# FishYuLi/BalancedGroupSoftmax

Measured on AMD Instinct MI355X. Metric: img/s fwd+bwd R50-FPN+BAGS 1333x800, 512 RoI (BASELINE metric: img/s/GPU fwd+bwd R50-FPN+BAGS 1333x800, 512 RoI; GroupSoftmax us/RoI), higher is better.
Workload: dtype f32 (conv/linear products on the bf16 MFMA from exact 3-way bf16 splits, fp32 accumulate: fp32-faithful)

## Files before the change

balancedgroupsoftmax_amd/capi.py:

```python
import ctypes
import os

_PKG = os.path.dirname(os.path.abspath(__file__))

c_i64p = ctypes.c_void_p
c_f32p = ctypes.c_void_p
c_ptr = ctypes.c_void_p

BGS_OK = 0
BGS_MAX_BINS = 16


class BgsLibraryError(RuntimeError):
    pass


class BgsCallError(RuntimeError):
    def __init__(self, fn, code, text):
        super().__init__('%s failed with code %d: %s' % (fn, code, text))
        self.code = code


SIGNATURES = {
    'bgs_version': (ctypes.c_int, []),
# ... 48 lines not shown
    'bgs_conv2d_dgrad_nhwc_f32': (ctypes.c_int, [c_f32p, c_f32p, c_f32p, c_f32p, c_f32p]
                                  + [ctypes.c_int] * 10 + [c_ptr]),
    'bgs_conv2d_wgrad_workspace_bytes': (ctypes.c_size_t, [ctypes.c_int] * 9),
    'bgs_conv2d_wgrad_nhwc_f32': (ctypes.c_int, [c_f32p, c_f32p, c_f32p, c_f32p]
                                  + [ctypes.c_int] * 10 + [c_ptr, c_ptr]),
    'bgs_fold_conv_bn_fwd': (ctypes.c_int, [c_f32p] * 6 + [ctypes.c_float] + [ctypes.c_int] * 5
                             + [c_f32p, c_f32p, c_ptr]),
    'bgs_fold_conv_bn_bwd': (ctypes.c_int, [c_f32p] * 7 + [ctypes.c_float] + [ctypes.c_int] * 5
                             + [c_f32p] * 4 + [c_ptr]),
    'bgs_conv2d_wgrad_bfx_workspace_bytes': (ctypes.c_size_t, [ctypes.c_int] * 9),
    'bgs_conv2d_wgrad_nhwc_f32_bfx': (ctypes.c_int, [c_f32p, c_f32p, c_f32p, c_f32p]
                                      + [ctypes.c_int] * 11 + [c_ptr, c_ptr]),
    'bgs_conv2d_wgrad_bfx_enable': (None, [ctypes.c_int]),
    'bgs_conv3x3_halo_nhwc_f32': (ctypes.c_int, [c_f32p, c_f32p, c_f32p, c_f32p] + [ctypes.c_int] * 6
                                  + [c_ptr]),
    'bgs_conv_bfx_weight_bytes': (ctypes.c_size_t, [ctypes.c_int, ctypes.c_int]),
    'bgs_conv_bfx_split_weights': (ctypes.c_int, [c_f32p, c_ptr, ctypes.c_int, ctypes.c_int, c_ptr]),
    'bgs_conv_dgrad_parity_enable': (None, [ctypes.c_int]),
    'bgs_conv_bfx_split_weights_dgrad': (ctypes.c_int, [c_f32p, c_ptr] + [ctypes.c_int] * 4 + [c_ptr]),
    'bgs_conv_bfx_workspace_bytes': (ctypes.c_size_t, [ctypes.c_longlong, ctypes.c_int, ctypes.c_int]),
    'bgs_conv2d_nhwc_f32_bfx_ws': (ctypes.c_int, [c_f32p, c_ptr, c_f32p, c_f32p, c_f32p]
                                   + [ctypes.c_int] * 12 + [c_ptr, ctypes.c_size_t, c_ptr]),
    'bgs_conv2d_dgrad_nhwc_f32_bfx_ws': (ctypes.c_int, [c_f32p, c_ptr, c_f32p, c_f32p, c_f32p]
                                         + [ctypes.c_int] * 11 + [c_ptr, ctypes.c_size_t, c_ptr]),
    'bgs_conv3x3_halo_bfx_workspace_bytes': (ctypes.c_size_t, [ctypes.c_int] * 5),
    'bgs_conv3x3_c3_fused_nhwc_f32_bfx': (ctypes.c_int, [c_f32p, c_ptr, c_f32p, c_ptr, c_f32p, c_f32p, c_f32p]
                                          + [ctypes.c_int] * 6 + [c_ptr]),
    'bgs_conv3x3_halo_nhwc_f32_bfx': (ctypes.c_int, [c_f32p, c_ptr, c_f32p, c_f32p]
                                      + [ctypes.c_int] * 7 + [c_ptr, ctypes.c_size_t, c_ptr]),
    'bgs_conv3x3_halo_nhwc_f32_bfx_ex': (ctypes.c_int, [c_f32p, c_ptr, c_f32p, c_f32p, c_f32p]
                                         + [ctypes.c_int] * 7 + [c_ptr, ctypes.c_size_t, c_ptr]),
    'bgs_conv3x3_planes_head_nhwc_f32_bfx': (ctypes.c_int, [c_f32p, c_ptr, c_f32p, c_ptr, c_f32p, c_f32p]
                                             + [ctypes.c_int] * 7 + [c_ptr]),
    'bgs_conv3x3_planes_head_eligible': (ctypes.c_int, [ctypes.c_int] * 6),
    'bgs_gs_loss_tuning': (None, [ctypes.c_int]),
    'bgs_gs_head_fold': (None, [ctypes.c_int]),
    'bgs_gs_loss_wavepriv_min_rows': (None, [ctypes.c_int]),
    'bgs_gs_merge_tuning': (None, [ctypes.c_int, ctypes.c_int]),
    'bgs_conv_bfx_wide_tuning': (None, [ctypes.c_int] * 3),
    'bgs_conv_bfx_wide_last_launch': (ctypes.c_int, []),
    'bgs_conv1x1_planes_enable': (None, [ctypes.c_int]),
    'bgs_conv1x1_planes_last_launch': (ctypes.c_int, []),
    'bgs_conv3x3_planes_enable': (None, [ctypes.c_int]),
    'bgs_conv3x3_planes_last_launch': (ctypes.c_int, []),
    'bgs_conv1x1_bres_enable': (None, [ctypes.c_int]),
    'bgs_conv1x1_bres_last_launch': (ctypes.c_int, []),
    'bgs_launch_census': (ctypes.c_int, [ctypes.c_int, ctypes.c_int]),
    'bgs_conv_bfx_tuning': (None, [ctypes.c_int] * 2),
    'bgs_conv_bfx_last_launch': (ctypes.c_int, [c_ptr, c_ptr]),
    'bgs_conv_tuning': (None, [ctypes.c_int] * 4),
    'bgs_conv_last_launch': (ctypes.c_int, [c_ptr, c_ptr, c_ptr, c_ptr]),
    'bgs_conv3x3_halo_bfx_tuning': (None, [ctypes.c_int] * 2),
    'bgs_conv3x3_halo_bfx_last_launch': (ctypes.c_int, [c_ptr, c_ptr]),
    'bgs_conv3x3_halo_bfx_last_wide': (ctypes.c_int, [c_ptr, c_ptr]),
    'bgs_conv3x3_halo_bfx_wide': (ctypes.c_int, [ctypes.c_int]),
    'bgs_grouped_conv3x3_nhwc_f32': (ctypes.c_int, [c_f32p, c_f32p, c_f32p, c_f32p] + [ctypes.c_int] * 7
                                     + [c_ptr]),
    'bgs_grouped_conv3x3_nhwc_bf16ops': (ctypes.c_int, [c_f32p, c_f32p, c_f32p, c_f32p] + [ctypes.c_int] * 7
                                         + [c_ptr]),
    'bgs_grouped_conv3x3_dgrad_nhwc_f32': (ctypes.c_int, [c_f32p, c_f32p, c_f32p] + [ctypes.c_int] * 6
                                           + [c_ptr]),
    'bgs_grouped_conv3x3_wgrad_workspace_bytes': (ctypes.c_size_t, [ctypes.c_int] * 6),
    'bgs_grouped_conv3x3_wgrad_nhwc_f32': (ctypes.c_int, [c_f32p, c_f32p, c_f32p, c_f32p]
                                           + [ctypes.c_int] * 7 + [c_ptr, c_ptr]),
    'bgs_deform_conv3x3_nhwc_f32': (ctypes.c_int, [c_f32p] * 5 + [ctypes.c_int] * 9 + [c_ptr]),
    'bgs_deform_conv3x3_dgrad_nhwc_f32': (ctypes.c_int, [c_f32p] * 6 + [ctypes.c_int] * 8 + [c_ptr]),
    'bgs_deform_conv3x3_wgrad_workspace_bytes': (ctypes.c_size_t, [ctypes.c_int] * 6),
    'bgs_deform_conv3x3_wgrad_nhwc_f32': (ctypes.c_int, [c_f32p] * 5 + [ctypes.c_int] * 9 + [c_ptr, c_ptr]),
    'bgs_sigmoid_focal_workspace_bytes': (ctypes.c_size_t, []),
    'bgs_sigmoid_focal_fwd': (ctypes.c_int, [c_f32p, ctypes.c_longlong, c_i64p, ctypes.c_int, ctypes.c_int,
                                             ctypes.c_float, ctypes.c_float, ctypes.c_int, c_f32p, c_ptr]),
    'bgs_sigmoid_focal_bwd': (ctypes.c_int, [c_f32p, ctypes.c_longlong, c_i64p, c_f32p, ctypes.c_int, ctypes.c_int,
                                             ctypes.c_float, ctypes.c_float, ctypes.c_int, c_f32p, c_ptr]),
    'bgs_sigmoid_focal_fwd_bwd': (ctypes.c_int, [c_f32p, ctypes.c_longlong, c_i64p, c_f32p, c_f32p, ctypes.c_int,
                                                 ctypes.c_int, ctypes.c_float, ctypes.c_float, ctypes.c_int, c_f32p,
                                                 ctypes.c_float, c_f32p, c_f32p, c_ptr, c_ptr]),
    'bgs_maxpool3x3s2_bwd_nhwc_f32': (ctypes.c_int, [c_f32p, c_f32p, c_f32p] + [ctypes.c_int] * 4 + [c_ptr]),
    'bgs_maxpool3x3s2_nhwc_f32': (ctypes.c_int, [c_f32p, c_f32p] + [ctypes.c_int] * 4 + [c_ptr]),
    'bgs_nchw_to_nhwc4_f32': (ctypes.c_int, [c_f32p, c_f32p] + [ctypes.c_int] * 4 + [c_ptr]),
    'bgs_conv2d_nhwc_bf16s': (ctypes.c_int, [c_ptr, c_ptr, c_f32p, c_ptr, ctypes.c_int, ctypes.c_int, c_ptr]
                              + [ctypes.c_int] * 11 + [c_ptr]),
    'bgs_grouped_conv3x3_nhwc_bf16s': (ctypes.c_int, [c_ptr, c_f32p, c_f32p, c_ptr] + [ctypes.c_int] * 7
                                       + [c_ptr]),
    'bgs_maxpool3x3s2_nhwc_f32_to_bf16': (ctypes.c_int, [c_f32p, c_ptr] + [ctypes.c_int] * 4 + [c_ptr]),
    'bgs_conv_bf16s_tuning': (None, [ctypes.c_int]),
    'bgs_roi_align_nhwc_fwd': (ctypes.c_int, [c_ptr, c_ptr, c_ptr, c_ptr, ctypes.c_int,
                                              ctypes.c_int, ctypes.c_float, c_f32p, ctypes.c_int,
                                              ctypes.c_int, ctypes.c_int, ctypes.c_int,
                                              ctypes.c_int, c_f32p, c_ptr, c_ptr]),
    'bgs_roi_align_nhwc_bwd': (ctypes.c_int, [c_ptr, c_ptr, c_ptr, c_ptr, ctypes.c_int,
                                              ctypes.c_int, ctypes.c_float, c_f32p, ctypes.c_int,
                                              ctypes.c_int, ctypes.c_int, ctypes.c_int,
                                              ctypes.c_int, c_f32p, c_ptr]),
    'bgs_roi_align_nhwc_fwd_f16': (ctypes.c_int, [c_ptr, c_ptr, c_ptr, c_ptr, ctypes.c_int,
                                                  ctypes.c_int, ctypes.c_float, c_f32p, ctypes.c_int,
                                                  ctypes.c_int, ctypes.c_int, ctypes.c_int,
                                                  ctypes.c_int, c_ptr, c_ptr, c_ptr]),
    'bgs_roi_align_nhwc_bwd_f16': (ctypes.c_int, [c_ptr, c_ptr, c_ptr, c_ptr, ctypes.c_int,
                                                  ctypes.c_int, ctypes.c_float, c_f32p, ctypes.c_int,
                                                  ctypes.c_int, ctypes.c_int, ctypes.c_int,
                                                  ctypes.c_int, c_ptr, c_ptr]),
    'bgs_roi_align_nhwc_fwd_ex': (ctypes.c_int, [c_ptr, c_ptr, c_ptr, c_ptr, ctypes.c_int,
                                                 ctypes.c_int, ctypes.c_float, c_f32p, ctypes.c_int,
                                                 ctypes.c_int, ctypes.c_int, ctypes.c_int,
                                                 ctypes.c_int, ctypes.c_int, ctypes.c_int, c_f32p,
                                                 c_ptr, c_ptr]),
    'bgs_roi_align_nhwc_bwd_ex': (ctypes.c_int, [c_ptr, c_ptr, c_ptr, c_ptr, ctypes.c_int,
                                                 ctypes.c_int, ctypes.c_float, c_f32p, ctypes.c_int,
                                                 ctypes.c_int, ctypes.c_int, ctypes.c_int,
                                                 ctypes.c_int, ctypes.c_int, c_f32p, c_ptr]),
    'bgs_resize_bilinear_nhwc_f32': (ctypes.c_int, [c_f32p, c_f32p] + [ctypes.c_int] * 7 + [c_ptr]),
    'bgs_resize_bilinear_nhwc_bwd_f32': (ctypes.c_int, [c_f32p, c_f32p] + [ctypes.c_int] * 7
                                         + [c_ptr]),
    'bgs_mask_target': (ctypes.c_int, [c_ptr, c_ptr, ctypes.c_int, ctypes.c_int, ctypes.c_int, c_f32p,
                                       ctypes.c_int, c_ptr, c_ptr, ctypes.c_int, ctypes.c_int, c_f32p,
                                       c_ptr]),
    'bgs_stem_fused_weight_bytes': (ctypes.c_size_t, []),
    'bgs_stem_fused_split_weights': (ctypes.c_int, [c_f32p, ctypes.c_int, c_ptr, c_ptr]),
    'bgs_stem_conv7x7s2_relu_maxpool_nchw_f32': (ctypes.c_int, [c_f32p, c_ptr, c_f32p, c_f32p, ctypes.c_int,
                                                                ctypes.c_int, ctypes.c_int, c_ptr]),
    'bgs_mask_paste_u8': (ctypes.c_int, [c_f32p, c_f32p, ctypes.c_int, ctypes.c_int, ctypes.c_int, ctypes.c_float,
                                         ctypes.c_float, ctypes.c_int, ctypes.c_int, c_ptr, c_ptr]),
    'bgs_mask_rle_workspace_bytes': (ctypes.c_size_t, [ctypes.c_int, ctypes.c_int]),
    'bgs_mask_rle_count': (ctypes.c_int, [c_f32p, c_f32p, ctypes.c_int, ctypes.c_int, ctypes.c_int, c_ptr, c_f32p,
                                          ctypes.c_float, ctypes.c_int, ctypes.c_int, c_ptr, ctypes.c_size_t, c_ptr,
                                          c_ptr]),
    'bgs_mask_rle_write': (ctypes.c_int, [c_f32p, c_f32p, ctypes.c_int, ctypes.c_int, ctypes.c_int, c_ptr, c_f32p,
                                          ctypes.c_float, ctypes.c_int, ctypes.c_int, c_ptr, ctypes.c_size_t, c_ptr,
                                          ctypes.c_longlong, c_ptr, c_ptr, c_ptr]),
    'bgs_rle_to_string': (ctypes.c_int, [c_ptr, c_ptr, ctypes.c_int, c_ptr, ctypes.c_longlong, c_ptr]),
    'bgs_rle_from_string': (ctypes.c_int, [c_ptr, c_ptr, ctypes.c_int, c_ptr, ctypes.c_longlong, c_ptr]),
    'bgs_lvis_box_iou': (ctypes.c_int, [c_ptr] * 5 + [ctypes.c_int] + [ctypes.c_longlong] * 3 + [c_ptr, c_ptr]),
    'bgs_lvis_rle_iou': (ctypes.c_int, [c_ptr] * 7 + [ctypes.c_int] + [ctypes.c_longlong] * 3 + [c_ptr, c_ptr]),
    'bgs_lvis_match_workspace_bytes': (ctypes.c_size_t, [ctypes.c_longlong, ctypes.c_int, ctypes.c_int]),
    'bgs_lvis_match': (ctypes.c_int, [c_ptr] * 4 + [ctypes.c_int] + [ctypes.c_longlong] * 2 + [c_ptr] * 4
                       + [c_ptr, ctypes.c_int, c_ptr, ctypes.c_int, c_ptr, ctypes.c_size_t] + [c_ptr] * 4 + [c_ptr]),
    'bgs_poly_rle_edge_points': (ctypes.c_int, [c_ptr, c_ptr, c_ptr, ctypes.c_longlong, ctypes.c_int, c_ptr, c_ptr]),
    'bgs_poly_rle_crossings': (ctypes.c_int, [c_ptr] * 4 + [ctypes.c_longlong, ctypes.c_int, ctypes.c_int, c_ptr, c_ptr,
                                              ctypes.c_longlong, c_ptr, c_ptr, c_ptr]),
    'bgs_poly_rle_events_from_transitions': (ctypes.c_int, [c_ptr] * 4 + [ctypes.c_int, ctypes.c_longlong, c_ptr,
                                                            c_ptr]),
    'bgs_poly_rle_events_from_runs': (ctypes.c_int, [c_ptr] * 3 + [ctypes.c_int, ctypes.c_longlong, c_ptr, c_ptr]),
    'bgs_poly_rle_resolve': (ctypes.c_int, [c_ptr] * 3 + [ctypes.c_int, ctypes.c_int] + [c_ptr] * 4
                             + [ctypes.c_int, ctypes.c_longlong] + [c_ptr] * 4),
    'bgs_poly_rle_write': (ctypes.c_int, [c_ptr] * 4 + [ctypes.c_int] + [c_ptr] * 4
                           + [ctypes.c_longlong, c_ptr, ctypes.c_longlong, c_ptr, c_ptr]),
    'bgs_mask_gt_logits': (ctypes.c_int, [c_f32p, c_f32p, c_f32p, c_ptr, ctypes.c_int, ctypes.c_int,
                                          ctypes.c_int, ctypes.c_int, c_f32p, c_ptr]),
    'bgs_mask_bce_partials': (ctypes.c_int, [ctypes.c_int]),
    'bgs_mask_bce': (ctypes.c_int, [c_f32p, c_f32p, c_f32p, c_ptr, c_f32p, c_ptr, c_f32p,
                                    ctypes.c_int, ctypes.c_int, ctypes.c_int, ctypes.c_int, c_f32p,
                                    c_f32p, c_f32p, c_f32p, c_ptr]),
    'bgs_topk_workspace_bytes': (ctypes.c_size_t, [ctypes.c_int, ctypes.c_int]),
    'bgs_topk_sorted_f32': (ctypes.c_int, [c_ptr, c_ptr, c_ptr, c_ptr, c_ptr, ctypes.c_int,
                                           ctypes.c_int, c_f32p, c_ptr, c_ptr, c_ptr]),
    'bgs_nms_workspace_bytes': (ctypes.c_size_t, [ctypes.c_int, ctypes.c_int]),
    'bgs_nms_batched': (ctypes.c_int, [c_f32p, c_ptr, ctypes.c_int, ctypes.c_int, ctypes.c_float,
                                       ctypes.c_int, ctypes.c_int, c_ptr, c_ptr, c_ptr, c_ptr]),
    'bgs_nms_merge_select': (ctypes.c_int, [c_f32p, c_ptr, c_ptr] + [ctypes.c_int] * 4 + [c_f32p, c_ptr, c_ptr]),
    'bgs_nms_gather': (ctypes.c_int, [c_f32p, c_ptr, c_ptr, ctypes.c_int, ctypes.c_int, c_f32p, c_f32p, c_ptr]),
    'bgs_soft_nms_batched': (ctypes.c_int, [c_f32p, c_ptr, ctypes.c_int, ctypes.c_int, ctypes.c_float, ctypes.c_int,
                                            ctypes.c_float, ctypes.c_float, c_ptr, c_f32p, c_ptr, c_ptr]),
    'bgs_det_candidates': (ctypes.c_int, [c_f32p, c_f32p, c_ptr, c_f32p] + [ctypes.c_int] * 4
                           + [ctypes.c_float, ctypes.c_int, c_f32p, c_ptr, c_ptr, c_ptr]),
    'bgs_det_select': (ctypes.c_int, [c_f32p, c_ptr, c_ptr, c_f32p, c_ptr] + [ctypes.c_int] * 4
                       + [c_f32p, c_ptr, c_ptr, c_ptr, c_ptr]),
    'bgs_gather_boxes': (ctypes.c_int, [c_f32p, c_ptr, c_f32p, ctypes.c_int, ctypes.c_int, ctypes.c_int, c_f32p,
                                        c_ptr, c_ptr]),
    'bgs_aug_map_boxes': (ctypes.c_int, [c_ptr, c_ptr] + [ctypes.c_int] * 4 + [c_ptr, c_ptr, c_ptr, ctypes.c_int,
                                                                               ctypes.c_int, c_f32p, c_f32p, c_ptr,
                                                                               c_ptr]),
    'bgs_aug_merge_bboxes': (ctypes.c_int, [c_ptr, c_ptr] + [ctypes.c_int] * 4 + [c_ptr, c_ptr, c_ptr, c_ptr, c_f32p,
                                                                                  c_f32p, c_ptr]),
    'bgs_aug_merge_masks': (ctypes.c_int, [c_ptr, c_ptr, ctypes.c_int, ctypes.c_int, ctypes.c_int, c_f32p, c_ptr]),
    'bgs_img_prep_u8': (ctypes.c_int, [c_ptr, c_ptr, ctypes.c_int, ctypes.c_int, c_f32p, ctypes.c_int, c_f32p,
                                       ctypes.c_int, ctypes.c_int, c_ptr]),
    'bgs_gt_mask_prep_u8': (ctypes.c_int, [c_ptr, c_ptr, ctypes.c_int, c_ptr, c_ptr, ctypes.c_longlong, c_ptr,
                                           ctypes.c_int, ctypes.c_int, c_ptr]),
    'bgs_gt_seg_prep_u8': (ctypes.c_int, [c_ptr, c_ptr, ctypes.c_int, c_ptr, ctypes.c_int, ctypes.c_int, c_ptr]),
    'bgs_iou_assign_workspace_bytes': (ctypes.c_size_t, [ctypes.c_int] * 3),
    'bgs_iou_assign': (ctypes.c_int, [c_f32p, ctypes.c_longlong, ctypes.c_int, c_ptr, c_f32p, c_ptr,
                                      ctypes.c_int, ctypes.c_int, ctypes.c_float, ctypes.c_float,
                                      ctypes.c_float, ctypes.c_float, c_ptr, c_f32p, c_ptr, c_ptr]),
    'bgs_rpn_loss_workspace_bytes': (ctypes.c_size_t, [ctypes.c_int] * 3),
    'bgs_rpn_loss': (ctypes.c_int, [c_ptr, c_ptr, ctypes.c_int, ctypes.c_int, c_f32p, c_ptr, c_ptr,
                                    c_ptr, c_f32p, c_ptr, ctypes.c_int, c_ptr, c_ptr,
                                    ctypes.c_float, ctypes.c_float, ctypes.c_float, ctypes.c_float,
                                    c_f32p, c_f32p, c_f32p, c_ptr, c_ptr]),
    'bgs_rpn_loss_grad': (ctypes.c_int, [c_ptr, c_ptr, c_ptr, ctypes.c_int, ctypes.c_int, c_f32p,
                                         c_ptr, c_ptr, c_ptr, c_f32p, c_ptr, ctypes.c_int, c_ptr,
                                         c_ptr, ctypes.c_float, ctypes.c_float, ctypes.c_float,
                                         ctypes.c_float, c_f32p, c_f32p, c_f32p, c_ptr]),
    'bgs_sample_pos_neg_workspace_bytes': (ctypes.c_size_t, [ctypes.c_int]),
    'bgs_sample_pos_neg': (ctypes.c_int, [c_ptr, ctypes.c_int, ctypes.c_int, ctypes.c_int, ctypes.c_float,
                                          ctypes.c_float, ctypes.c_uint64, c_ptr, c_ptr, c_ptr, c_ptr,
                                          c_ptr]),
    'bgs_sample_rois': (ctypes.c_int, [c_ptr, c_ptr, ctypes.c_int, ctypes.c_int, ctypes.c_float,
                                       ctypes.c_uint64, c_ptr, c_ptr, c_ptr, c_ptr, c_ptr]),
    'bgs_sample_rois_ex': (ctypes.c_int, [c_ptr, c_ptr, c_ptr, ctypes.c_int, ctypes.c_int, ctypes.c_float,
                                          ctypes.c_uint64, c_ptr, c_ptr, c_ptr, c_ptr, c_ptr, c_ptr, c_ptr]),
    'bgs_random_keys': (ctypes.c_int, [ctypes.c_uint64, c_ptr, ctypes.c_int, c_ptr, c_ptr]),
    'bgs_decode_proposals': (ctypes.c_int, [c_ptr, c_ptr, c_ptr, ctypes.c_int, ctypes.c_int, c_f32p,
                                            c_ptr, c_f32p, ctypes.c_int, c_ptr, c_ptr, c_ptr,
                                            ctypes.c_float, ctypes.c_int, c_f32p, c_ptr]),
    'bgs_refine_boxes': (ctypes.c_int, [c_f32p, c_ptr, c_f32p, ctypes.c_int, ctypes.c_int, c_ptr,
                                        ctypes.c_int, c_f32p, c_f32p, ctypes.c_float, c_f32p, c_ptr]),
    'bgs_rcnn_targets': (ctypes.c_int, [c_ptr, c_ptr, c_ptr, c_ptr, c_ptr, c_ptr, c_f32p, c_ptr,
                                        ctypes.c_int, ctypes.c_int, c_ptr, c_ptr, ctypes.c_float,
                                        c_f32p, c_ptr, c_f32p, c_f32p, c_f32p, c_ptr]),
}

_LIB = None


def lib_filename():
    variant = os.environ.get('BGS_LIB_VARIANT', '')
    return 'libbgs_%s.so' % variant if variant else 'libbgs.so'


def lib_path():
    return os.environ.get('BGS_LIB_PATH', os.path.join(_PKG, lib_filename()))


def load():
    global _LIB
    if _LIB is not None:
        return _LIB
    path = lib_path()
    if not os.path.exists(path):
        raise BgsLibraryError(
            '%s not found. Build the HIP kernels first: '
            '`python -m balancedgroupsoftmax_amd.csrc.build` (or __graft_entry__.build()). '
            'There is deliberately no CPU fallback.' % path)
    try:
        lib = ctypes.CDLL(path)
    except OSError as e:
        raise BgsLibraryError('cannot load %s: %s' % (path, e))
    for name, (res, args) in SIGNATURES.items():
        try:
            fn = getattr(lib, name)
        except AttributeError:
            raise BgsLibraryError('%s does not export %s (stale build?)' % (path, name))
        fn.restype = res
        fn.argtypes = args
    _LIB = lib
    return lib


def check(fn_name, code):
    if code != BGS_OK:
        raise BgsCallError(fn_name, code, load().bgs_error_string(code).decode())


def host_i64(a):
    import numpy as np
    a = np.ascontiguousarray(a, dtype=np.int64)
    return a, a.ctypes.data_as(ctypes.c_void_p)


def ptr(t):
    return None if t is None else t.data_ptr()


_RAW_STREAM = []


def raw_stream(device=None):
    import torch
    if not _RAW_STREAM:
        _RAW_STREAM.append(getattr(torch._C, '_cuda_getCurrentRawStream', None))
    idx = device if isinstance(device, int) else getattr(device, 'index', None)
    if idx is None:
        if isinstance(device, str):
            idx = torch.device(device).index
        if idx is None:
            idx = torch.cuda.current_device()
    fn = _RAW_STREAM[0]
    if fn is None:
        return torch.cuda.current_stream(idx).cuda_stream
    return fn(idx)


def current_stream(device=None):
    return raw_stream(device)
```

balancedgroupsoftmax_amd/csrc/det_targets.hip:

```cpp
#include <math.h>
#include <string.h>

#include "bgs_common.h"

namespace {

constexpr int kMaxImgs = 16;
constexpr int kMaxLevels = 8;
constexpr int kGtChunk = 256;

struct ImgTable {
  int gt_off[kMaxImgs + 1];
  int img_h[kMaxImgs], img_w[kMaxImgs];
};

__device__ __forceinline__ float iou1(float ax1, float ay1, float ax2, float ay2, float aarea,
                                      float bx1, float by1, float bx2, float by2) {
#pragma clang fp contract(off)
  const float w = fmaxf(fminf(ax2, bx2) - fmaxf(ax1, bx1) + 1.f, 0.f);
  const float h = fmaxf(fminf(ay2, by2) - fmaxf(ay1, by1) + 1.f, 0.f);
  const float ov = w * h;
  const float barea = (bx2 - bx1 + 1.f) * (by2 - by1 + 1.f);
  return ov / (barea + aarea - ov);
}
// ... 310 lines not shown
  const size_t row = ((size_t)n * Lv.hw[lvl] + loc) * ch;
  const float* o = Lv.out[lvl] + row;
  float* d_o = G.dout[lvl] + row;
  const float inv = 1.f / num_total[0];
  const float x = o[a];
  const float t = ps ? 1.f : 0.f;
  const float w = ps ? pos_weight : 1.f;
  const float sig = 1.f / (1.f + expf(-x));
  d_o[a] = g_cls[lvl] * w_cls * w * (sig - t) * inv;
  if (ps) {
    const int g = T.gt_off[n] + assigned[(size_t)n * A + i] - 1;
    const float* an = anchors + (size_t)i * 4;
    const float* gb = gt + (size_t)g * 4;
    float d[4];
    encode_delta(an[0], an[1], an[2], an[3], gb[0], gb[1], gb[2], gb[3], cod, d);
    const float sc = g_bbox[lvl] * w_bbox * inv;
#pragma unroll
    for (int c = 0; c < 4; ++c) {
      const float df = o[na + a * 4 + c] - d[c];
      const float ad = fabsf(df);
      const float gr = ad < beta ? df / beta : (df > 0.f ? 1.f : (df < 0.f ? -1.f : 0.f));
      d_o[na + a * 4 + c] = sc * gr;
    }
  }
}

struct CountTable {
  int count[kMaxLevels];
};

__global__ __launch_bounds__(256) void decode_proposals_kernel(
    LevelTable Lv, ImgTable T, CountTable Ct, const float* __restrict__ anchors,
    const long long* __restrict__ top_idx, const float* __restrict__ top_logit, Coding cod,
    float max_ratio, int nmax, float* __restrict__ boxes_out) {
  const int n = blockIdx.z, l = blockIdx.y;
  const int j = blockIdx.x * 256 + threadIdx.x;
  if (j >= nmax) return;
  float* o = boxes_out + (((size_t)n * Lv.num_levels + l) * nmax + j) * 5;
  if (j >= Ct.count[l]) {
    o[0] = o[1] = o[2] = o[3] = o[4] = 0.f;
    return;
  }
  const size_t tj = ((size_t)n * Lv.num_levels + l) * nmax + j;
  long long p = top_idx[tj];
  const int na = Lv.num_anchors, ch = 5 * na;
  const long long cnt = (long long)Lv.hw[l] * na;
  p = p < 0 ? 0 : (p >= cnt ? cnt - 1 : p);
  const int loc = (int)(p / na), a = (int)(p - (long long)loc * na);
  const float* src = Lv.out[l] + ((size_t)n * Lv.hw[l] + loc) * ch + na + a * 4;
  const float* an = anchors + ((size_t)Lv.start[l] + p) * 4;
  const float dx = src[0] * cod.stdv[0] + cod.mean[0];
  const float dy = src[1] * cod.stdv[1] + cod.mean[1];
  float dw = src[2] * cod.stdv[2] + cod.mean[2];
  float dh = src[3] * cod.stdv[3] + cod.mean[3];
  dw = fminf(fmaxf(dw, -max_ratio), max_ratio);
  dh = fminf(fmaxf(dh, -max_ratio), max_ratio);
  const float px = (an[0] + an[2]) * 0.5f, py = (an[1] + an[3]) * 0.5f;
  const float pw = an[2] - an[0] + 1.f, ph = an[3] - an[1] + 1.f;
  const float gw = pw * expf(dw), gh = ph * expf(dh);
  const float gx = px + pw * dx, gy = py + ph * dy;
  const float wmax = (float)(T.img_w[n] - 1), hmax = (float)(T.img_h[n] - 1);
  o[0] = fminf(fmaxf(gx - gw * 0.5f + 0.5f, 0.f), wmax);
  o[1] = fminf(fmaxf(gy - gh * 0.5f + 0.5f, 0.f), hmax);
  o[2] = fminf(fmaxf(gx + gw * 0.5f - 0.5f, 0.f), wmax);
  o[3] = fminf(fmaxf(gy + gh * 0.5f - 0.5f, 0.f), hmax);
  o[4] = 1.f / (1.f + expf(-top_logit[tj]));
}

__global__ __launch_bounds__(256) void refine_boxes_kernel(const float* __restrict__ rois,
                                                           const long long* __restrict__ labels,
                                                           const float* __restrict__ bbox_pred,
                                                           int K, int pred_cols, Coding cod,
                                                           ImgTable T, int n_img, float max_ratio,
                                                           float* __restrict__ out) {
#pragma clang fp contract(off)
  const int k = blockIdx.x * 256 + threadIdx.x;
  if (k >= K) return;
  const float* r = rois + (size_t)k * 5;
  int img = (int)r[0];
  img = img < 0 ? 0 : (img >= n_img ? n_img - 1 : img);
  long long c = 0;
  if (pred_cols > 4 && labels) {
    c = labels[k];
    const long long nc = pred_cols / 4;
    c = c < 0 ? 0 : (c >= nc ? nc - 1 : c);
  }
  const float* d = bbox_pred + (size_t)k * pred_cols + c * 4;
  const float dx = d[0] * cod.stdv[0] + cod.mean[0];
  const float dy = d[1] * cod.stdv[1] + cod.mean[1];
  float dw = d[2] * cod.stdv[2] + cod.mean[2];
  float dh = d[3] * cod.stdv[3] + cod.mean[3];
  dw = fminf(fmaxf(dw, -max_ratio), max_ratio);
  dh = fminf(fmaxf(dh, -max_ratio), max_ratio);
  const float pw = r[3] - r[1] + 1.0f, ph = r[4] - r[2] + 1.0f;
  const float px = (r[1] + r[3]) * 0.5f, py = (r[2] + r[4]) * 0.5f;
  const float gw = pw * expf(dw), gh = ph * expf(dh);
  const float gx = px + pw * dx, gy = py + ph * dy;
  const float wmax = (float)(T.img_w[img] - 1), hmax = (float)(T.img_h[img] - 1);
  float* o = out + (size_t)k * 4;
  o[0] = fminf(fmaxf(gx - gw * 0.5f + 0.5f, 0.f), wmax);
  o[1] = fminf(fmaxf(gy - gh * 0.5f + 0.5f, 0.f), hmax);
  o[2] = fminf(fmaxf(gx + gw * 0.5f - 0.5f, 0.f), wmax);
  o[3] = fminf(fmaxf(gy + gh * 0.5f - 0.5f, 0.f), hmax);
}

struct PtrTable {
  const float* boxes[kMaxImgs];
  const int* assigned[kMaxImgs];
  const long long* inds[kMaxImgs];
  const uint8_t* valid[kMaxImgs];
  const long long* gt_labels[kMaxImgs];
  int box_stride[kMaxImgs];
};

__global__ __launch_bounds__(256) void rcnn_targets_kernel(PtrTable P, ImgTable T,
                                                           const float* __restrict__ gt, Coding cod,
                                                           int num, float pos_weight,
                                                           float* __restrict__ rois,
                                                           long long* __restrict__ labels,
                                                           float* __restrict__ label_weights,
                                                           float* __restrict__ bbox_targets,
                                                           float* __restrict__ bbox_weights) {
  const int n = blockIdx.y;
  const int j = blockIdx.x * 256 + threadIdx.x;
  if (j >= num) return;
  const size_t r = (size_t)n * num + j;
  const long long ci = P.inds[n][j];
  const float* b = P.boxes[n] + (size_t)ci * P.box_stride[n];
  const int a = P.assigned[n][ci];
  const bool ok = P.valid[n] ? P.valid[n][j] != 0 : true;
  const bool pos = ok && a > 0;
  rois[r * 5 + 0] = (float)n;
  rois[r * 5 + 1] = b[0];
  rois[r * 5 + 2] = b[1];
  rois[r * 5 + 3] = b[2];
  rois[r * 5 + 4] = b[3];
  float d[4] = {0.f, 0.f, 0.f, 0.f};
  long long lab = 0;
  if (pos) {
    const int g = T.gt_off[n] + (int)a - 1;
    const float* gb = gt + (size_t)g * 4;
    encode_delta(b[0], b[1], b[2], b[3], gb[0], gb[1], gb[2], gb[3], cod, d);
    lab = P.gt_labels[n][a - 1];
  }
  labels[r] = lab;
  label_weights[r] = pos ? pos_weight : (ok ? 1.f : 0.f);
#pragma unroll
  for (int c = 0; c < 4; ++c) {
    bbox_targets[r * 4 + c] = d[c];
    bbox_weights[r * 4 + c] = pos ? 1.f : 0.f;
  }
}

int fill_img_table(ImgTable* T, const int* host_gt_offsets, const int* host_img_hw, int N) {
  if (N <= 0 || N > kMaxImgs || !host_gt_offsets) return BGS_ERR_INVALID_ARG;
  for (int i = 0; i <= kMaxImgs; ++i) T->gt_off[i] = 0;
  for (int i = 0; i <= N; ++i) T->gt_off[i] = host_gt_offsets[i];
  for (int i = 0; i < kMaxImgs; ++i) {
    T->img_h[i] = host_img_hw ? host_img_hw[2 * (i < N ? i : 0)] : 1;
    T->img_w[i] = host_img_hw ? host_img_hw[2 * (i < N ? i : 0) + 1] : 1;
  }
  for (int i = 0; i < N; ++i)
    if (T->gt_off[i + 1] < T->gt_off[i]) return BGS_ERR_INVALID_ARG;
  return BGS_OK;
}

int fill_level_table(LevelTable* Lv, const float* const* host_outs, const int* host_hw, int L,
                     int num_anchors) {
  if (L <= 0 || L > kMaxLevels || !host_outs || !host_hw || num_anchors <= 0)
    return BGS_ERR_INVALID_ARG;
  int start = 0;
  for (int l = 0; l < kMaxLevels; ++l) {
    Lv->out[l] = l < L ? host_outs[l] : nullptr;
    Lv->hw[l] = l < L ? host_hw[l] : 0;
    Lv->start[l] = start;
    if (l < L) {
      if (!host_outs[l] || host_hw[l] <= 0) return BGS_ERR_INVALID_ARG;
      start += host_hw[l] * num_anchors;
    }
  }
  Lv->start[kMaxLevels] = start;
  for (int l = L; l <= kMaxLevels; ++l) Lv->start[l] = start;
  Lv->num_levels = L;
  Lv->num_anchors = num_anchors;
  return BGS_OK;
}

}

extern "C" size_t bgs_iou_assign_workspace_bytes(int N, int A, int G_total) {
  if (N <= 0 || A <= 0 || G_total < 0) return 0;
  const size_t g = (size_t)(G_total > 0 ? G_total : 1);
  return (size_t)N * A * 4 + (size_t)N * g * 4 + (size_t)N * ((A + 255) / 256) * g * 4;
}

extern "C" int bgs_iou_assign(const float* boxes, long long box_img_stride, int box_stride,
                              const uint8_t* valid,
                              const float* gt, const int* host_gt_offsets, int N, int A,
                              float pos_iou_thr, float neg_iou_lo, float neg_iou_hi,
                              float min_pos_iou, int* assigned, float* max_overlaps_out,
                              void* workspace, bgs_stream_t stream) {
  if (N <= 0 || A <= 0 || !boxes || !gt || !assigned || !workspace || box_stride < 4)
    return BGS_ERR_INVALID_ARG;
  ImgTable T;
  const int rc = fill_img_table(&T, host_gt_offsets, nullptr, N);
  if (rc != BGS_OK) return rc;
  const int Gt = T.gt_off[N];
  if (Gt <= 0) return BGS_ERR_INVALID_ARG;
  hipStream_t st = (hipStream_t)stream;
  float* box_max = max_overlaps_out;
  int* gt_max = (int*)((char*)workspace + (size_t)N * A * 4);
  int* blk_max = gt_max + (size_t)N * Gt;
  const size_t ng = (size_t)N * Gt;
  hipLaunchKernelGGL(fill_i32_kernel, dim3((unsigned)((ng + 255) / 256)), dim3(256), 0, st, gt_max,
                     (int)0xBF800000 , ng);
  dim3 grid((unsigned)((A + 255) / 256), (unsigned)N);
  const float send = min_pos_iou > 0.f ? min_pos_iou : 0.f;
  int send_bits;
  memcpy(&send_bits, &send, sizeof(int));
  hipLaunchKernelGGL(iou_gtmax_kernel, grid, dim3(256), 0, st, boxes, box_img_stride, box_stride,
                     valid, gt, T, A, Gt, pos_iou_thr, neg_iou_lo, neg_iou_hi, send_bits, box_max, blk_max,
                     gt_max, assigned);
  hipLaunchKernelGGL(iou_assign_kernel, grid, dim3(256), 0, st, boxes, box_img_stride, box_stride,
                     valid, gt, T, A, Gt, blk_max, gt_max, min_pos_iou, assigned);
  BGS_RETURN_LAUNCH_STATUS();
}

extern "C" size_t bgs_rpn_loss_workspace_bytes(int N, int A_total, int L) {
  if (N <= 0 || A_total <= 0 || L <= 0) return 0;
  return (size_t)N * ((A_total + 255) / 256) * L * 4 * sizeof(float);
}

extern "C" int bgs_rpn_loss(const float* const* host_level_outs, const int* host_level_hw, int L,
                            int num_anchors, const float* anchors, const int* assigned,
                            const uint8_t* pos_mask, const uint8_t* neg_mask, const float* gt,
                            const int* host_gt_offsets, int N, const float* host_means,
                            const float* host_stds, float beta, float pos_weight,
                            float loss_weight_cls, float loss_weight_bbox, float* loss_cls_out,
                            float* loss_bbox_out, float* num_total_out, void* workspace,
                            bgs_stream_t stream) {
  if (!anchors || !assigned || !pos_mask || !neg_mask || !gt || !loss_cls_out || !loss_bbox_out ||
      !workspace || !host_means || !host_stds || !(beta > 0.f))
    return BGS_ERR_INVALID_ARG;
  LevelTable Lv;
  int rc = fill_level_table(&Lv, host_level_outs, host_level_hw, L, num_anchors);
  if (rc != BGS_OK) return rc;
  ImgTable T;
  rc = fill_img_table(&T, host_gt_offsets, nullptr, N);
  if (rc != BGS_OK) return rc;
  Coding cod;
  for (int c = 0; c < 4; ++c) {
    cod.mean[c] = host_means[c];
    cod.stdv[c] = host_stds[c];
  }
  const int A = Lv.start[kMaxLevels];
  const int blocks = (A + 255) / 256;
  hipStream_t st = (hipStream_t)stream;
  hipLaunchKernelGGL(rpn_loss_kernel, dim3(blocks, N), dim3(256), 0, st, Lv, T, anchors, assigned,
                     pos_mask, neg_mask, gt, cod, beta, pos_weight <= 0.f ? 1.f : pos_weight, A,
                     (float*)workspace);
  hipLaunchKernelGGL(rpn_loss_finalize_kernel, dim3(1), dim3(1024), 0, st, (const float*)workspace,
                     Lv, N, blocks, L, loss_weight_cls, loss_weight_bbox, loss_cls_out, loss_bbox_out,
                     num_total_out);
  BGS_RETURN_LAUNCH_STATUS();
}

__global__ __launch_bounds__(256) void random_keys_kernel(uint64_t seed,
                                                          const long long* __restrict__ draw, int n,
                                                          long long* __restrict__ out) {
  const int i = blockIdx.x * 256 + threadIdx.x;
  if (i >= n) return;
  const uint64_t d = draw ? (uint64_t)draw[0] : 0ull;
  uint64_t x = seed + 0x9E3779B97F4A7C15ull * ((uint64_t)i + 1ull) + 0xD1B54A32D192ED03ull * (d + 1ull);
  x ^= x >> 30; x *= 0xBF58476D1CE4E5B9ull;
  x ^= x >> 27; x *= 0x94D049BB133111EBull;
  x ^= x >> 31;
  out[i] = (long long)(x >> 2);
}

extern "C" int bgs_random_keys(uint64_t seed, const long long* draw_counter, int n, long long* out,
                               bgs_stream_t stream) {
  if (n < 0) return BGS_ERR_INVALID_ARG;
  if (n == 0) return BGS_OK;
  if (!out) return BGS_ERR_INVALID_ARG;
  hipLaunchKernelGGL(random_keys_kernel, dim3((n + 255) / 256), dim3(256), 0, (hipStream_t)stream,
                     seed, draw_counter, n, out);
  BGS_RETURN_LAUNCH_STATUS();
}

extern "C" int bgs_rpn_loss_grad(const float* const* host_level_outs,
                                 float* const* host_level_douts, const int* host_level_hw, int L,
                                 int num_anchors, const float* anchors, const int* assigned,
                                 const uint8_t* pos_mask, const uint8_t* neg_mask, const float* gt,
                                 const int* host_gt_offsets, int N, const float* host_means,
                                 const float* host_stds, float beta, float pos_weight,
                                 float loss_weight_cls, float loss_weight_bbox,
                                 const float* num_total, const float* grad_loss_cls,
                                 const float* grad_loss_bbox, bgs_stream_t stream) {
  if (!anchors || !assigned || !pos_mask || !neg_mask || !gt || !num_total || !grad_loss_cls ||
      !grad_loss_bbox || !host_level_douts || !host_means || !host_stds || !(beta > 0.f))
    return BGS_ERR_INVALID_ARG;
  LevelTable Lv;
  int rc = fill_level_table(&Lv, host_level_outs, host_level_hw, L, num_anchors);
  if (rc != BGS_OK) return rc;
  GradTable G;
  for (int l = 0; l < kMaxLevels; ++l) G.dout[l] = nullptr;
  for (int l = 0; l < L; ++l) {
    if (!host_level_douts[l]) return BGS_ERR_INVALID_ARG;
    G.dout[l] = host_level_douts[l];
  }
  ImgTable T;
  rc = fill_img_table(&T, host_gt_offsets, nullptr, N);
  if (rc != BGS_OK) return rc;
  Coding cod;
  for (int c = 0; c < 4; ++c) {
    cod.mean[c] = host_means[c];
    cod.stdv[c] = host_stds[c];
  }
  const int A = Lv.start[kMaxLevels];
  const int blocks = (A + 255) / 256;
  hipLaunchKernelGGL(rpn_loss_grad_kernel, dim3(blocks, N), dim3(256), 0, (hipStream_t)stream, Lv,
                     G, T, anchors, assigned, pos_mask, neg_mask, gt, cod, beta,
                     pos_weight <= 0.f ? 1.f : pos_weight, A, num_total, loss_weight_cls,
                     loss_weight_bbox, grad_loss_cls, grad_loss_bbox);
  BGS_RETURN_LAUNCH_STATUS();
}

extern "C" int bgs_decode_proposals(const float* const* host_level_outs, const int* host_level_hw,
                                    const int* host_level_counts, int L, int num_anchors,
                                    const float* anchors, const long long* top_idx,
                                    const float* top_logit, int N, const int* host_img_hw,
                                    const float* host_means, const float* host_stds,
                                    float wh_ratio_clip, int nmax, float* boxes_out,
                                    bgs_stream_t stream) {
  if (!anchors || !top_idx || !top_logit || !boxes_out || !host_img_hw || !host_means ||
      !host_stds || !host_level_counts || nmax <= 0 || !(wh_ratio_clip > 0.f))
    return BGS_ERR_INVALID_ARG;
  LevelTable Lv;
  int rc = fill_level_table(&Lv, host_level_outs, host_level_hw, L, num_anchors);
  if (rc != BGS_OK) return rc;
  ImgTable T;
  int zero_off[kMaxImgs + 1] = {0};
  rc = fill_img_table(&T, zero_off, host_img_hw, N);
  if (rc != BGS_OK) return rc;
  Coding cod;
  CountTable Ct;
  for (int c = 0; c < 4; ++c) {
    cod.mean[c] = host_means[c];
    cod.stdv[c] = host_stds[c];
  }
  for (int l = 0; l < kMaxLevels; ++l) Ct.count[l] = l < L ? host_level_counts[l] : 0;
  hipLaunchKernelGGL(decode_proposals_kernel, dim3((nmax + 255) / 256, L, N), dim3(256), 0,
                     (hipStream_t)stream, Lv, T, Ct, anchors, top_idx, top_logit, cod,
                     fabsf(logf(wh_ratio_clip)), nmax, boxes_out);
  BGS_RETURN_LAUNCH_STATUS();
}

extern "C" int bgs_refine_boxes(const float* rois, const long long* labels, const float* bbox_pred,
                                int K, int pred_cols, const int* host_img_hw, int N,
                                const float* host_means, const float* host_stds, float wh_ratio_clip,
                                float* out, bgs_stream_t stream) {
  if (K < 0 || N <= 0 || N > kMaxImgs || pred_cols < 4 || pred_cols % 4 != 0) return BGS_ERR_INVALID_ARG;
  if (K == 0) return BGS_OK;
  if (!rois || !bbox_pred || !out || !host_img_hw || !host_means || !host_stds || wh_ratio_clip <= 0.f)
    return BGS_ERR_INVALID_ARG;
  if (pred_cols > 4 && !labels) return BGS_ERR_INVALID_ARG;
  ImgTable T;
  for (int i = 0; i < kMaxImgs; ++i) {
    const int s = i < N ? i : 0;
    T.gt_off[i] = 0;
    T.img_h[i] = host_img_hw[2 * s];
    T.img_w[i] = host_img_hw[2 * s + 1];
  }
  T.gt_off[kMaxImgs] = 0;
  Coding cod;
  for (int i = 0; i < 4; ++i) {
    cod.mean[i] = host_means[i];
    cod.stdv[i] = host_stds[i];
  }
  hipLaunchKernelGGL(refine_boxes_kernel, dim3((K + 255) / 256), dim3(256), 0, (hipStream_t)stream, rois,
                     labels, bbox_pred, K, pred_cols, cod, T, N, fabsf(logf(wh_ratio_clip)), out);
  BGS_RETURN_LAUNCH_STATUS();
}

extern "C" int bgs_rcnn_targets(const float* const* host_boxes, const int* host_box_strides,
                                const int* const* host_assigned,
                                const long long* const* host_inds,
                                const uint8_t* const* host_valid,
                                const long long* const* host_gt_labels, const float* gt,
                                const int* host_gt_offsets, int N, int num, const float* host_means,
                                const float* host_stds, float pos_weight, float* rois,
                                long long* labels, float* label_weights, float* bbox_targets,
                                float* bbox_weights, bgs_stream_t stream) {
  if (!host_boxes || !host_box_strides || !host_assigned || !host_inds || !host_gt_labels || !gt ||
      !rois || !labels || !label_weights || !bbox_targets || !bbox_weights || num <= 0 ||
      !host_means || !host_stds)
    return BGS_ERR_INVALID_ARG;
  ImgTable T;
  const int rc = fill_img_table(&T, host_gt_offsets, nullptr, N);
  if (rc != BGS_OK) return rc;
  PtrTable P;
  for (int i = 0; i < kMaxImgs; ++i) {
    const int s = i < N ? i : 0;
    P.boxes[i] = host_boxes[s];
    P.assigned[i] = host_assigned[s];
    P.inds[i] = host_inds[s];
    P.valid[i] = host_valid ? host_valid[s] : nullptr;
    P.gt_labels[i] = host_gt_labels[s];
    P.box_stride[i] = host_box_strides[s];
    if (i < N && (!P.boxes[i] || !P.assigned[i] || !P.inds[i] || !P.gt_labels[i] ||
                  P.box_stride[i] < 4))
      return BGS_ERR_INVALID_ARG;
  }
  Coding cod;
  for (int c = 0; c < 4; ++c) {
    cod.mean[c] = host_means[c];
    cod.stdv[c] = host_stds[c];
  }
  hipLaunchKernelGGL(rcnn_targets_kernel, dim3((num + 255) / 256, N), dim3(256), 0,
                     (hipStream_t)stream, P, T, gt, cod, num, pos_weight <= 0.f ? 1.f : pos_weight,
                     rois, labels, label_weights, bbox_targets, bbox_weights);
  BGS_RETURN_LAUNCH_STATUS();
}
```

balancedgroupsoftmax_amd/csrc/topk.hip:

```cpp
#include "bgs_common.h"

namespace {

constexpr int kMaxProblems = 64;
constexpr int kMaxK = 4096;
constexpr int kBins = 2048;
constexpr int kChunk = 4096;
constexpr int kState = 8;

struct TopkProblems {
  const float* row[kMaxProblems];
  int len[kMaxProblems];
  int k[kMaxProblems];
  int inner[kMaxProblems];
  int pitch[kMaxProblems];
};

__device__ __forceinline__ float topk_elem(const TopkProblems& pr, int p, const float* row, int i) {
  const int inner = pr.inner[p];
  if (inner == 0) return row[i];
  const int q = i / inner;
  return row[(size_t)q * pr.pitch[p] + (i - q * inner)];
}

struct TopkWs {
  int* hist;
  unsigned* state;
  unsigned long long* list;
};

__device__ __forceinline__ unsigned key_of(float f) {
  const unsigned b = __float_as_uint(f);
  return (b & 0x80000000u) ? ~b : (b | 0x80000000u);
}
__device__ __forceinline__ float value_of(unsigned key) {
  return __uint_as_float((key & 0x80000000u) ? (key & 0x7fffffffu) : ~key);
}

__device__ __forceinline__ int shift_of(int pass) { return pass == 0 ? 21 : (pass == 1 ? 10 : 0); }
__device__ __forceinline__ int bins_of(int pass) { return pass == 2 ? 1024 : 2048; }

__device__ __forceinline__ void topk_pick(const int* __restrict__ g, int nb, int k_rem, int* s_wave, int* s_res,
                                          int& digit, int& k_in) {
  const int tid = threadIdx.x, lane = tid & 63, wave = tid >> 6;
  const int per = nb / 256;
  int cnt[8];
  int mine = 0;
#pragma unroll
  for (int j = 0; j < 8; ++j) {
    cnt[j] = j < per ? g[nb - 1 - (tid * per + j)] : 0;
    mine += cnt[j];
  }
  int incl = mine;
#pragma unroll
  for (int off = 1; off < 64; off <<= 1) {
    const int t = __shfl_up(incl, off, 64);
    if (lane >= off) incl += t;
  }
  if (lane == 63) s_wave[wave] = incl;
  __syncthreads();
  int base = 0;
  for (int w = 0; w < wave; ++w) base += s_wave[w];
  incl += base;
  const int excl = incl - mine;
  if (excl < k_rem && k_rem <= incl) {
    int c = excl, d = 0;
#pragma unroll
    for (int j = 0; j < 8; ++j) {
      if (j < per) {
        if (k_rem <= c + cnt[j]) {
          d = nb - 1 - (tid * per + j);
          break;
        }
        c += cnt[j];
      }
    }
    s_res[0] = d;
    s_res[1] = k_rem - c;
  }
  __syncthreads();
  digit = s_res[0];
  k_in = s_res[1];
  __syncthreads();
}

__global__ __launch_bounds__(256) void topk_hist_kernel(TopkProblems pr, TopkWs ws, int pass) {
  __shared__ int h[kBins];
  __shared__ int s_wave[4], s_res[2];
  const int p = blockIdx.y, tid = threadIdx.x;
  const int len = pr.len[p];
  const int lo = blockIdx.x * kChunk;
  if (lo >= len) return;
  const int hi = min(len, lo + kChunk);
  const int k = min(pr.k[p], len);
  if (k <= 0) return;
  const int nb = bins_of(pass), shift = shift_of(pass);
  for (int b = tid; b < nb; b += 256) h[b] = 0;
  unsigned* st = ws.state + p * kState;
  unsigned prefix = 0, pmask = 0;
  if (pass > 0) {
    int k_rem = k;
    if (pass == 2) {
      prefix = st[0];
      pmask = st[1];
      k_rem = (int)st[2];
    }
    int digit, k_in;
    topk_pick(ws.hist + ((size_t)p * 3 + (pass - 1)) * kBins, bins_of(pass - 1), k_rem, s_wave, s_res, digit, k_in);
    prefix |= (unsigned)digit << shift_of(pass - 1);
    pmask |= (unsigned)(bins_of(pass - 1) - 1) << shift_of(pass - 1);
    if (blockIdx.x == 0 && tid == 0) {
      unsigned* o = st + (pass == 1 ? 0 : 5);
      o[0] = prefix;
      o[1] = pmask;
      o[2] = (unsigned)k_in;
    }
  }
  __syncthreads();
  const float* row = pr.row[p];
  for (int i = lo + tid; i < hi; i += 256) {
    const unsigned key = key_of(topk_elem(pr, p, row, i));
    if ((key & pmask) == prefix) atomicAdd(&h[(key >> shift) & (nb - 1)], 1);
  }
  __syncthreads();
  int* g = ws.hist + ((size_t)p * 3 + pass) * kBins;
  for (int b = tid; b < nb; b += 256)
    if (h[b]) atomicAdd(&g[b], h[b]);
}

__global__ __launch_bounds__(256) void topk_collect_kernel(TopkProblems pr, TopkWs ws, int kmax) {
  const int p = blockIdx.y, tid = threadIdx.x;
  const int len = pr.len[p];
  const int lo = blockIdx.x * kChunk;
  if (lo >= len) return;
  const int hi = min(len, lo + kChunk);
  const int k = min(pr.k[p], len);
  unsigned* st = ws.state + p * kState;
  unsigned long long* list = ws.list + (size_t)p * kmax;
  const float* row = pr.row[p];
  if (k <= 0) return;
  __shared__ int s_wave[4], s_res[2];
  int digit, need_eq;
  topk_pick(ws.hist + ((size_t)p * 3 + 2) * kBins, bins_of(2), (int)st[7], s_wave, s_res, digit, need_eq);
  const unsigned T = st[5] | ((unsigned)digit << shift_of(2));
  const int lane = tid & 63;
  const unsigned long long below = (1ull << lane) - 1ull;
  constexpr int kLg = 512, kLe = 256;
  __shared__ unsigned long long s_g[kLg], s_e[kLe];
  __shared__ int s_n[2], s_base[2];
  if (tid < 2) s_n[tid] = 0;
  __syncthreads();
  for (int i0 = lo; i0 < hi; i0 += 256) {
    const int i = i0 + tid;
    const bool in = i < hi;
    const unsigned key = in ? key_of(topk_elem(pr, p, row, i)) : 0u;
    const unsigned long long comp = ((unsigned long long)key << 32) | (0xffffffffu - (unsigned)i);
    const bool gt = in && key > T, eq = in && key == T;
    const unsigned long long mg = __ballot(gt), me = __ballot(eq);
    if (mg) {
      const int leader = __ffsll((long long)mg) - 1;
      int base = 0;
      if (lane == leader) base = atomicAdd(&s_n[0], __popcll(mg));
      base = __shfl(base, leader, 64);
      const int slot = base + __popcll(mg & below);
      if (gt) {
        if (slot < kLg) s_g[slot] = comp;
        else list[atomicAdd(&st[3], 1u)] = comp;
      }
    }
    if (me) {
      const int leader = __ffsll((long long)me) - 1;
      int base = 0;
      if (lane == leader) base = atomicAdd(&s_n[1], __popcll(me));
      base = __shfl(base, leader, 64);
      const int slot = base + __popcll(me & below);
      if (eq) {
        if (slot < kLe) s_e[slot] = comp;
        else {
          const int g = (int)atomicAdd(&st[4], 1u);
          if (g < need_eq) list[k - 1 - g] = comp;
        }
      }
    }
  }
  __syncthreads();
  const int ng = min(s_n[0], kLg), ne = min(s_n[1], kLe);
  if (tid == 0) {
    s_base[0] = ng ? (int)atomicAdd(&st[3], (unsigned)ng) : 0;
    s_base[1] = ne ? (int)atomicAdd(&st[4], (unsigned)ne) : 0;
  }
  __syncthreads();
  for (int i = tid; i < ng; i += 256) list[s_base[0] + i] = s_g[i];
  for (int i = tid; i < ne; i += 256) {
    const int g = s_base[1] + i;
    if (g < need_eq) list[k - 1 - g] = s_e[i];
  }
}

__global__ __launch_bounds__(1024) void topk_sort_kernel(TopkProblems pr, TopkWs ws, int kmax,
                                                         float* __restrict__ out_val,
                                                         long long* __restrict__ out_idx) {
  __shared__ unsigned long long buf[kMaxK];
  const int p = blockIdx.x, tid = threadIdx.x;
  const int k = min(pr.k[p], pr.len[p]);
  int m = 1;
  while (m < k) m <<= 1;
  const unsigned long long* list = ws.list + (size_t)p * kmax;
  for (int i = tid; i < m; i += 1024) buf[i] = i < k ? list[i] : 0ull;
  __syncthreads();
  for (int size = 2; size <= m; size <<= 1) {
    for (int stride = size >> 1; stride > 0; stride >>= 1) {
      for (int j = tid; j < (m >> 1); j += 1024) {
        const int lo = (j / stride) * (stride << 1) + (j % stride);
        const int hi = lo + stride;
        const bool desc = ((lo & size) == 0);
        const unsigned long long a = buf[lo], b = buf[hi];
        if ((a < b) == desc) {
          buf[lo] = b;
          buf[hi] = a;
        }
      }
      bgs::bitonic_stage_sync(size, stride);
    }
  }
  __syncthreads();
  float* ov = out_val + (size_t)p * kmax;
  long long* oi = out_idx + (size_t)p * kmax;
  for (int i = tid; i < kmax; i += 1024) {
    if (i < k) {
      const unsigned long long c = buf[i];
      ov[i] = value_of((unsigned)(c >> 32));
      oi[i] = (long long)(0xffffffffu - (unsigned)(c & 0xffffffffu));
    } else {
      ov[i] = 0.f;
      oi[i] = 0;
    }
  }
}

}

extern "C" size_t bgs_topk_workspace_bytes(int P, int kmax) {
  if (P <= 0 || kmax <= 0) return 0;
  return (size_t)P * (3 * kBins * sizeof(int) + kState * sizeof(unsigned) +
                      (size_t)kmax * sizeof(unsigned long long));
}

extern "C" int bgs_topk_sorted_f32(const float* const* host_rows, const int* host_len,
                                   const int* host_k, const int* host_inner,
                                   const int* host_pitch, int P, int kmax, float* out_val,
                                   long long* out_idx, void* workspace, bgs_stream_t stream) {
  if (P < 0 || kmax <= 0) return BGS_ERR_INVALID_ARG;
  if (P == 0) return BGS_OK;
  if (!host_rows || !host_len || !host_k || !out_val || !out_idx || !workspace)
    return BGS_ERR_INVALID_ARG;
  if (P > kMaxProblems || kmax > kMaxK) return BGS_ERR_UNSUPPORTED;
  TopkProblems pr;
  int maxlen = 0;
  for (int p = 0; p < kMaxProblems; ++p) {
    pr.row[p] = nullptr;
    pr.len[p] = pr.k[p] = pr.inner[p] = pr.pitch[p] = 0;
  }
  if ((host_inner == nullptr) != (host_pitch == nullptr)) return BGS_ERR_INVALID_ARG;
  for (int p = 0; p < P; ++p) {
    if (host_len[p] < 0 || host_k[p] < 0 || host_k[p] > kmax) return BGS_ERR_INVALID_ARG;
    if (host_len[p] > 0 && !host_rows[p]) return BGS_ERR_INVALID_ARG;
    pr.row[p] = host_rows[p];
    pr.len[p] = host_len[p];
    pr.k[p] = host_k[p];
    if (host_inner) {
      if (host_inner[p] < 0 || (host_inner[p] > 0 && host_pitch[p] < host_inner[p]))
        return BGS_ERR_INVALID_ARG;
      pr.inner[p] = host_inner[p];
      pr.pitch[p] = host_pitch[p];
    }
    if (host_len[p] > maxlen) maxlen = host_len[p];
  }
  TopkWs ws;
  ws.hist = reinterpret_cast<int*>(workspace);
  ws.state = reinterpret_cast<unsigned*>(ws.hist + (size_t)P * 3 * kBins);
  ws.list = reinterpret_cast<unsigned long long*>(ws.state + (size_t)P * kState);
  hipStream_t st = (hipStream_t)stream;
  if (hipMemsetAsync(workspace, 0, (size_t)P * (3 * kBins * sizeof(int) + kState * sizeof(unsigned)),
                     st) != hipSuccess)
    return BGS_ERR_LAUNCH;
  const int G = maxlen > 0 ? (maxlen + kChunk - 1) / kChunk : 1;
  for (int pass = 0; pass < 3; ++pass)
    hipLaunchKernelGGL(topk_hist_kernel, dim3(G, P), dim3(256), 0, st, pr, ws, pass);
  hipLaunchKernelGGL(topk_collect_kernel, dim3(G, P), dim3(256), 0, st, pr, ws, kmax);
  hipLaunchKernelGGL(topk_sort_kernel, dim3(P), dim3(1024), 0, st, pr, ws, kmax, out_val, out_idx);
  BGS_RETURN_LAUNCH_STATUS();
}
```

balancedgroupsoftmax_amd/detectors.py:

```python
import torch
import torch.nn as nn

from . import box_ops, builder, merge_augs
from . import functional as BF
from . import post_processing as PP
from .registry import DETECTORS


_GT_ROWS = {}


def _gt_index_row(G, device):
    key = (int(G), str(device))
    t = _GT_ROWS.get(key)
    if t is None:
        if len(_GT_ROWS) > 4096:
            _GT_ROWS.clear()
        t = _GT_ROWS[key] = torch.arange(1, int(G) + 1, device=device, dtype=torch.int32)
    return t


@DETECTORS.register_module
class TwoStageDetector(nn.Module):

    def __init__(self, backbone, neck=None, shared_head=None, rpn_head=None,
                 bbox_roi_extractor=None, bbox_head=None, mask_roi_extractor=None, mask_head=None,
                 train_cfg=None, test_cfg=None, pretrained=None):
        super().__init__()
        if shared_head is not None:
            raise NotImplementedError('shared_head (C4 heads) is not on the BAGS path')
        self.backbone = builder.build_backbone(backbone)
        self.neck = builder.build_neck(neck) if neck is not None else None
        self.rpn_head = builder.build_head(rpn_head) if rpn_head is not None else None
        self.bbox_roi_extractor = builder.build_roi_extractor(bbox_roi_extractor) \
            if bbox_head is not None else None
        self.bbox_head = builder.build_head(bbox_head) if bbox_head is not None else None
        self.mask_head = None
        if mask_head is not None:
            if mask_roi_extractor is not None:
                self.mask_roi_extractor = builder.build_roi_extractor(mask_roi_extractor)
                self.share_roi_extractor = False
            else:
                self.share_roi_extractor = True
                self.mask_roi_extractor = self.bbox_roi_extractor
            self.mask_head = builder.build_head(mask_head)
        self.train_cfg, self.test_cfg = train_cfg, test_cfg
        self.fp16_enabled = False
        self.init_weights(pretrained=pretrained)

    with_neck = property(lambda self: self.neck is not None)
    with_rpn = property(lambda self: self.rpn_head is not None)
    with_bbox = property(lambda self: self.bbox_head is not None)
    with_mask = property(lambda self: self.mask_head is not None)
    with_shared_head = property(lambda self: False)

    def init_weights(self, pretrained=None):
        self.backbone.init_weights(pretrained=pretrained)
        if self.with_neck:
            self.neck.init_weights()
        if self.with_rpn:
            self.rpn_head.init_weights()
        if self.with_bbox:
            self.bbox_roi_extractor.init_weights()
            self.bbox_head.init_weights()
        if self.with_mask:
            self.mask_head.init_weights()
            if not self.share_roi_extractor:
                self.mask_roi_extractor.init_weights()

    def extract_feat(self, img):
        x = self.backbone(img)
        return self.neck(x) if self.with_neck else x

    def _sample_rois_fused(self, proposal_list, gt_bboxes, gt_labels, samplers=None, rc=None,
                           head=None):
        rc = self.train_cfg.rcnn if rc is None else rc
        ac, sc = rc.assigner, rc.sampler
        N = len(proposal_list)
        if hasattr(proposal_list, 'batched'):
            props, pv = proposal_list.batched
            props = props.contiguous()
            pvalid = (pv.view(torch.uint8) if pv.dtype == torch.bool else pv.to(torch.uint8)).contiguous()
        else:
            props = torch.stack([p for p, _ in proposal_list]).contiguous()
            pvalid = torch.stack([v for _, v in proposal_list]).to(torch.uint8).contiguous()
        gt_cat = torch.cat([g[:, :4] for g in gt_bboxes]).float().contiguous()
        offs = [0]
        for g in gt_bboxes:
            offs.append(offs[-1] + int(g.size(0)))
        assigned = BF.iou_assign(props, gt_cat, offs, ac.pos_iou_thr, ac.neg_iou_thr,
                                 ac.get('min_pos_iou', 0.0), valid=pvalid, shared_boxes=False)
        add_gt = sc.get('add_gt_as_proposals', True)
        rcnn_hook = samplers.get('rcnn') if samplers else None
        boxes_l, assigned_l, inds_l, valid_l = [], [], [], []
        for i in range(N):
            b, a = props[i, :, :4], assigned[i]
            if add_gt:
                G = gt_bboxes[i].size(0)
                b = torch.cat([gt_bboxes[i][:, :4].float(), b], 0)
                a = torch.cat([_gt_index_row(G, a.device), a])
            boxes_l.append(b.contiguous())
            assigned_l.append(a.contiguous())
            if rcnn_hook is not None:
                inds, _, valid = rcnn_hook(a, sc.num, sc.pos_fraction)
                inds_l.append(inds.contiguous())
                valid_l.append(valid)
        if rcnn_hook is None:
            if any(a.numel() > 4096 for a in assigned_l):
                raise NotImplementedError('bgs_sample_rois sorts <= 4096 candidates per image in LDS '
                                          '(rpn_proposal.max_num + GT boxes)')
            need_extra = self.with_mask or isinstance(self.bbox_head, nn.ModuleList)
            res = BF.sample_rois(assigned_l, sc.num, sc.pos_fraction,
                                 gt_counts=[int(g.size(0)) if add_gt else 0 for g in gt_bboxes]
                                 if need_extra else None)
            inds_all, valid_all = res[0], res[2].view(torch.bool)
            inds_l = [inds_all[i] for i in range(N)]
            valid_l = [valid_all[i] for i in range(N)]
            if need_extra:
                self._sampled_gt_inds = res[3]
                self._sampled_valid = valid_all
                self._sampled_is_gt = res[4].view(torch.bool)
        if rcnn_hook is not None and (self.with_mask or isinstance(self.bbox_head, nn.ModuleList)):
            self._sampled_gt_inds = torch.stack(
                [assigned_l[i].gather(0, inds_l[i]).to(torch.int32) - 1 for i in range(N)])
            self._sampled_valid = torch.stack(valid_l)
            self._sampled_is_gt = torch.stack(
                [(inds_l[i] < gt_bboxes[i].size(0)) if add_gt else torch.zeros_like(valid_l[i])
                 for i in range(N)])
        head = self.bbox_head if head is None else head
        rois, labels, lw, bt, bw = BF.rcnn_targets(
            boxes_l, assigned_l, inds_l, valid_l, [g.contiguous() for g in gt_labels], gt_cat, offs,
            sc.num, head.target_means, head.target_stds, rc.pos_weight)
        return rois, (labels, lw, bt, bw)

    def _rpn_forward_train(self, x, img_meta, gt_bboxes, proposals, samplers, losses, fork_loss=False):
        if not self.with_rpn:
            return [(p, torch.ones(p.size(0), dtype=torch.bool, device=p.device)) for p in proposals]
        cls_scores, bbox_preds = self.rpn_head(x)
        self._rpn_loss_fork = None
        if fork_loss and cls_scores[0].is_cuda and BF.rpn_loss_fork_enabled() and not samplers and \
                not (torch.is_grad_enabled() and cls_scores[0].requires_grad):
            with BF.forked(cls_scores[0].device, lane=1) as fk:
                losses.update(self.rpn_head.loss(cls_scores, bbox_preds, gt_bboxes, img_meta,
                                                 self.train_cfg.rpn, samplers=samplers))
            fk.hold(cls_scores, bbox_preds, self.rpn_head._fused, gt_bboxes)
            self._rpn_loss_fork = fk
        else:
            losses.update(self.rpn_head.loss(cls_scores, bbox_preds, gt_bboxes, img_meta,
                                             self.train_cfg.rpn, samplers=samplers))
        proposal_cfg = self.train_cfg.get('rpn_proposal', None)
        if proposal_cfg is None:
            proposal_cfg = self.test_cfg.rpn
        proposal_list = self.rpn_head.get_bboxes(cls_scores, bbox_preds, img_meta, proposal_cfg)
        if samplers is not None and 'proposals' in samplers:
            self._own_proposals = proposal_list
            proposal_list = samplers['proposals'](proposal_list)
        self.rpn_head._fused = None
        return proposal_list

    def _join_rpn_loss(self):
        fk = getattr(self, '_rpn_loss_fork', None)
        if fk is not None:
            fk.join()
            self._rpn_loss_fork = None

    def trunk_is_frozen(self):
        mods = [self.backbone] + ([self.neck] if self.with_neck else [])
        return not any(p.requires_grad for m in mods for p in m.parameters())

    def forward_train(self, img, img_meta, gt_bboxes, gt_labels, gt_bboxes_ignore=None,
                      gt_masks=None, proposals=None, samplers=None, feats=None):
        x = self.extract_feat(img) if feats is None else feats
        losses = dict()
        proposal_list = self._rpn_forward_train(x, img_meta, gt_bboxes, proposals, samplers, losses,
                                                fork_loss=True)
        if self.with_bbox:
            if not self.train_cfg.rcnn.assigner.get('gt_max_assign_all', True):
                raise NotImplementedError('gt_max_assign_all=False')
            rois, targets = self._sample_rois_fused(proposal_list, gt_bboxes, gt_labels, samplers)
            mask_fk = None
            if self.with_mask and rois.is_cuda and BF.rpn_loss_fork_enabled() and not (
                    torch.is_grad_enabled() and any(p.requires_grad for p in self.mask_head.parameters())):
                with BF.forked(rois.device, lane=2) as mask_fk:
                    mask_losses = self._mask_forward_train(x, rois, targets[0], gt_masks, img.size(0))
                mask_fk.hold(x, rois, targets, gt_masks)
            bbox_feats = self.bbox_roi_extractor(x[:self.bbox_roi_extractor.num_inputs], rois)
            cls_score, bbox_pred = self.bbox_head(bbox_feats, nhwc=True, reg_labels=targets[0])
            losses.update(self.bbox_head.loss(cls_score, bbox_pred, *targets))
            if mask_fk is not None:
                mask_fk.join()
                losses.update(mask_losses)
            elif self.with_mask:
                losses.update(self._mask_forward_train(x, rois, targets[0], gt_masks, img.size(0)))
        elif self.with_mask:
            losses.update(self._mask_forward_train(x, rois, targets[0], gt_masks, img.size(0)))
        self._join_rpn_loss()
        return losses

    def _mask_forward_train(self, x, rois, labels, gt_masks, num_imgs):
        if gt_masks is None:
            raise ValueError('the mask branch needs gt_masks (per image a uint8 [G, H, W] tensor)')
        if not rois.is_cuda:
            raise NotImplementedError('the mask branch runs on the GPU path only')
        sc = self.train_cfg.rcnn.sampler
        max_pos = int(sc.num * sc.pos_fraction)
        num = sc.num
        sel = (torch.arange(num_imgs, device=rois.device).view(-1, 1) * num +
               torch.arange(max_pos, device=rois.device).view(1, -1)).reshape(-1)
        pos_rois = rois[sel].contiguous()
        pos_labels = labels[sel].contiguous()
        valid = pos_labels > 0
        gt_inds = self._sampled_gt_inds[:, :max_pos].reshape(-1).contiguous()
        masks = [torch.as_tensor(m).to(device=rois.device, dtype=torch.uint8).contiguous()
                 for m in gt_masks]
        if self.share_roi_extractor:
            raise NotImplementedError('share_roi_extractor=True (7x7 features for the mask head) '
                                      'is not used by the BAGS configs')
        mask_feats = self.mask_roi_extractor(x[:self.mask_roi_extractor.num_inputs], pos_rois)
        feats = self.mask_head.features(mask_feats, nhwc=True)
        mask_targets = self.mask_head.get_target_fixed(pos_rois, gt_inds, valid, masks,
                                                       self.train_cfg.rcnn)
        return self.mask_head.loss_from_features(feats, mask_targets, pos_labels, valid)

    _last_bbox_head = property(lambda self: self.bbox_head)
    _segm_head = property(lambda self: self.mask_head)

    def _check_test_cfg(self):
        """What the detector's test_cfg asks for and is not built (raised before any device work)."""

    def _test_context(self, x):
        return None

    def _box_scores(self, x, ctx, rois, img_metas, batched=False):
        feats = self.bbox_roi_extractor(x[:self.bbox_roi_extractor.num_inputs], rois)
        return (rois,) + tuple(self.bbox_head(feats, nhwc=True))

    def _stage_mask_probs(self, x, ctx, rois, labels):
        feats = self.mask_roi_extractor(x[:self.mask_roi_extractor.num_inputs], rois)
        return [self.mask_head.get_mask_probs(self.mask_head.features(feats, nhwc=True), labels)]

    def _mask_probs(self, x, ctx, rois, labels):
        if rois.shape[0] == 0:
            return rois.new_zeros((0, 28, 28))
        probs = self._stage_mask_probs(x, ctx, rois, labels)
        return probs[0] if len(probs) == 1 else sum(probs) / float(len(probs))

    @staticmethod
    def _image_proposals(proposal_list, as_rois=True):
        props, valid = proposal_list[0] if isinstance(proposal_list[0], tuple) else (proposal_list[0], None)
        if as_rois:
            props = torch.cat([props.new_zeros((props.size(0), 1)), props[:, :4]], dim=1)
        return props, valid

    @staticmethod
    def _check_segm(segm):
        if segm not in (None, 'rle'):
            raise ValueError("segm: None (mask probabilities) or 'rle' (the reference's segm_results), got %r" % (segm,))
        return segm is not None

    def simple_test_rpn(self, x, img_meta, rpn_test_cfg):
        cls_scores, bbox_preds = self.rpn_head(x)
        return self.rpn_head.get_bboxes(cls_scores, bbox_preds, img_meta, rpn_test_cfg)

    def simple_test_bboxes(self, x, img_meta, proposals, rcnn_test_cfg, rescale=False, ctx=None):
        rois, valid = self._image_proposals(proposals)
        rois, cls_score, bbox_pred = self._box_scores(x, ctx, rois, img_meta)
        bboxes, scores = self._last_bbox_head.get_det_bboxes(
            rois, cls_score, bbox_pred, img_meta[0]['img_shape'], img_meta[0]['scale_factor'],
            rescale=rescale, cfg=None)
        if valid is not None:
            scores = torch.where(valid[:, None], scores, scores.new_full((), -1.0))
        det_bboxes, det_labels = PP.multiclass_nms(bboxes, scores, rcnn_test_cfg.score_thr,
                                                   rcnn_test_cfg.nms, rcnn_test_cfg.max_per_img)
        return det_bboxes, det_labels, scores

    def simple_test_mask(self, x, img_meta, det_bboxes, det_labels, rescale=False, paste=False, encode=None,
                         ctx=None):
        if paste and det_bboxes.shape[0] == 0:
            return [[] for _ in range(self._segm_head.num_classes - 1)]
        boxes = det_bboxes[:, :4] * img_meta[0]['scale_factor'] if rescale else det_bboxes[:, :4]
        rois = torch.cat([boxes.new_zeros((boxes.size(0), 1)), boxes], dim=1)
        probs = self._mask_probs(x, ctx, rois, det_labels)
# ... 477 lines not shown
```

balancedgroupsoftmax_amd/functional.py:

```python
import ctypes
import itertools
import os

import torch

from . import capi

_WS = {}


def _workspace(nbytes, device):
    key = (device.index, capi.raw_stream(device))
    buf = _WS.get(key)
    if buf is None or buf.numel() < nbytes:
        buf = torch.empty(max(int(nbytes), 1 << 20), dtype=torch.uint8, device=device)
        _WS[key] = buf
    return buf


def reset_workspaces():
    _WS.clear()


_SIDE = {}
# ... 1514 lines not shown
    _require_cuda(rois, *feats)
    lib = capi.load()
    L = len(feats)
    N, _, _, C = feats[0].shape
    for f in feats:
        assert f.dtype == torch.float32 and f.is_contiguous() and f.shape[0] == N and f.shape[3] == C
    rois = _f32c(rois)
    K = rois.shape[0]
    ph, pw = (out_size, out_size) if isinstance(out_size, int) else tuple(out_size)
    accumulate = out is not None
    if accumulate:
        assert tuple(out.shape) == (K, ph, pw, C) and out.is_contiguous() and \
            out.dtype == torch.float32, (out.shape, (K, ph, pw, C))
    else:
        out = torch.empty((K, ph, pw, C), dtype=torch.float32, device=rois.device)
    lv = torch.empty((K,), dtype=torch.int32, device=rois.device) if return_levels else None
    ptrs = (ctypes.c_void_p * L)(*[f.data_ptr() for f in feats])
    hs = (ctypes.c_int * L)(*[int(f.shape[1]) for f in feats])
    ws = (ctypes.c_int * L)(*[int(f.shape[2]) for f in feats])
    sc = (ctypes.c_float * L)(*[1.0 / s for s in featmap_strides])
    rc = lib.bgs_roi_align_nhwc_fwd_ex(ptrs, hs, ws, sc, L, N, float(finest_scale), capi.ptr(rois),
                                       K, C, ph, pw, sample_num, int(pool), int(accumulate),
                                       capi.ptr(out), capi.ptr(lv),
                                       capi.current_stream(rois.device))
    capi.check('bgs_roi_align_nhwc_fwd_ex', rc)
    return (out, lv) if return_levels else out


def roi_align_nhwc_bwd(dout, rois, dfeats, featmap_strides, sample_num=2, finest_scale=56, pool=1):
    import ctypes
    _require_cuda(dout, rois, *dfeats)
    lib = capi.load()
    L = len(dfeats)
    N, _, _, C = dfeats[0].shape
    for f in dfeats:
        assert f.dtype == torch.float32 and f.is_contiguous() and f.shape[0] == N and f.shape[3] == C
    rois = _f32c(rois)
    dout = _f32c(dout)
    K, ph, pw, C2 = dout.shape
    assert C2 == C and rois.shape[0] == K
    ptrs = (ctypes.c_void_p * L)(*[f.data_ptr() for f in dfeats])
    hs = (ctypes.c_int * L)(*[int(f.shape[1]) for f in dfeats])
    ws = (ctypes.c_int * L)(*[int(f.shape[2]) for f in dfeats])
    sc = (ctypes.c_float * L)(*[1.0 / s for s in featmap_strides])
    rc = lib.bgs_roi_align_nhwc_bwd_ex(ptrs, hs, ws, sc, L, N, float(finest_scale), capi.ptr(rois),
                                       K, C, ph, pw, sample_num, int(pool), capi.ptr(dout),
                                       capi.current_stream(rois.device))
    capi.check('bgs_roi_align_nhwc_bwd_ex', rc)
    return dfeats


class _RoIAlignFn(torch.autograd.Function):

    @staticmethod
    def forward(ctx, rois, strides, out_size, sample_num, finest_scale, pool, base, *feats):
        ctx.save_for_backward(rois)
        ctx.cfg = (tuple(strides), sample_num, finest_scale, pool, [tuple(f.shape) for f in feats],
                   base is not None)
        if base is not None:
            ctx.mark_dirty(base)
        return roi_align_nhwc([f.detach() for f in feats], rois, strides, out_size, sample_num,
                              finest_scale, pool=pool, out=base)

    @staticmethod
    @torch.autograd.function.once_differentiable
    def backward(ctx, dout):
        rois, = ctx.saved_tensors
        strides, sample_num, finest_scale, pool, shapes, has_base = ctx.cfg
        dout = dout.contiguous()
        dfeats = [None] * len(shapes)
        if any(ctx.needs_input_grad[7:]):
            dfeats = [torch.zeros(s, dtype=torch.float32, device=dout.device) for s in shapes]
            roi_align_nhwc_bwd(dout, rois, dfeats, strides, sample_num, finest_scale, pool=pool)
        dbase = dout if has_base and ctx.needs_input_grad[6] else None
        return (None, None, None, None, None, None, dbase) + tuple(dfeats)


def roi_align_nhwc_autograd(feats, rois, featmap_strides, out_size=7, sample_num=2,
                            finest_scale=56, pool=1, add_to=None):
    ts = list(feats) + ([add_to] if add_to is not None else [])
    if torch.is_grad_enabled() and any(t.requires_grad for t in ts):
        return _RoIAlignFn.apply(rois, tuple(featmap_strides), out_size, sample_num, finest_scale,
                                 pool, add_to, *feats)
    return roi_align_nhwc(feats, rois, featmap_strides, out_size, sample_num, finest_scale,
                          pool=pool, out=add_to)


def resize_bilinear_nhwc(x, size):
    _require_cuda(x)
    lib = capi.load()
    assert x.dtype == torch.float32 and x.is_contiguous() and x.dim() == 4
    N, H, W, C = x.shape
    Ho, Wo = int(size[0]), int(size[1])
    y = torch.empty((N, Ho, Wo, C), dtype=torch.float32, device=x.device)
    rc = lib.bgs_resize_bilinear_nhwc_f32(capi.ptr(x), capi.ptr(y), N, H, W, C, Ho, Wo, 1,
                                          capi.current_stream(x.device))
    capi.check('bgs_resize_bilinear_nhwc_f32', rc)
    return y


class _ResizeBilinearFn(torch.autograd.Function):

    @staticmethod
    def forward(ctx, x, size):
        ctx.in_shape = tuple(x.shape)
        return resize_bilinear_nhwc(x.detach(), size)

    @staticmethod
    @torch.autograd.function.once_differentiable
    def backward(ctx, dy):
        lib = capi.load()
        N, H, W, C = ctx.in_shape
        dy = dy.contiguous()
        dx = torch.zeros(ctx.in_shape, dtype=torch.float32, device=dy.device)
        rc = lib.bgs_resize_bilinear_nhwc_bwd_f32(capi.ptr(dy), capi.ptr(dx), N, H, W, C,
                                                  dy.shape[1], dy.shape[2], 1,
                                                  capi.current_stream(dy.device))
        capi.check('bgs_resize_bilinear_nhwc_bwd_f32', rc)
        return dx, None


def resize_bilinear_nhwc_autograd(x, size):
    if torch.is_grad_enabled() and x.requires_grad:
        return _ResizeBilinearFn.apply(x, tuple(size))
    return resize_bilinear_nhwc(x, size)


def topk_sorted(rows, ks, kmax, inner=None):
    import ctypes
    _require_cuda(*rows)
    lib = capi.load()
    N = rows[0].shape[0]
    L = len(rows)
    dev = rows[0].device
    ptrs, lens, kk, inn, pit = [], [], [], [], []
    for i in range(N):
        for r, k in zip(rows, ks):
            assert r.shape[0] == N and r.dtype == torch.float32 and r.is_contiguous()
            per = r[0].numel()
            ptrs.append(r.data_ptr() + i * per * 4)
            if inner is None:
                lens.append(per)
                inn.append(0)
                pit.append(0)
            else:
                C = int(r.shape[-1])
                lens.append(per // C * int(inner))
                inn.append(int(inner))
                pit.append(C)
            kk.append(int(k))
    P = N * L
    vals = torch.empty((N, L, kmax), dtype=torch.float32, device=dev)
    idx = torch.empty((N, L, kmax), dtype=torch.int64, device=dev)
    ws = _workspace(lib.bgs_topk_workspace_bytes(P, int(kmax)), dev)
    rc = lib.bgs_topk_sorted_f32((ctypes.c_void_p * P)(*ptrs), _c_int_array(lens), _c_int_array(kk),
                                 _c_int_array(inn) if inner is not None else None,
                                 _c_int_array(pit) if inner is not None else None,
                                 P, int(kmax), capi.ptr(vals), capi.ptr(idx), capi.ptr(ws),
                                 capi.current_stream(dev))
    capi.check('bgs_topk_sorted_f32', rc)
    return vals, idx


def nms_batched(boxes, counts, iou_thr, iou_mode=0, max_keep=0):
    _require_cuda(boxes, counts)
    lib = capi.load()
    boxes = _f32c(boxes)
    assert boxes.dim() == 3 and boxes.shape[2] == 5 and counts.dtype == torch.int32
    P, nmax, _ = boxes.shape
    dev = boxes.device
    keep = torch.empty((P, nmax), dtype=torch.int32, device=dev)
    keep_count = torch.empty((P,), dtype=torch.int32, device=dev)
    ws = _workspace(lib.bgs_nms_workspace_bytes(P, nmax), dev)
    rc = lib.bgs_nms_batched(capi.ptr(boxes), capi.ptr(counts), P, nmax, float(iou_thr),
                             int(iou_mode), int(max_keep), capi.ptr(keep), capi.ptr(keep_count),
                             capi.ptr(ws), capi.current_stream(dev))
    capi.check('bgs_nms_batched', rc)
    return keep, keep_count


SOFT_NMS_METHODS = {'hard': 0, 'linear': 1, 'gaussian': 2}


def soft_nms_batched(dets, counts, iou_thr, method='linear', sigma=0.5, min_score=1e-3):
    _require_cuda(dets, counts)
    code = SOFT_NMS_METHODS.get(method, method)
    if code not in (0, 1, 2):
        raise ValueError('Invalid method for SoftNMS: {}'.format(method))
    lib = capi.load()
    dets = _f32c(dets)
    assert dets.dim() == 3 and dets.shape[2] == 5 and counts.dtype == torch.int32
    P, nmax, _ = dets.shape
    dev = dets.device
    order = torch.empty((P, nmax), dtype=torch.int32, device=dev)
    scores = torch.empty((P, nmax), dtype=torch.float32, device=dev)
    keep_count = torch.empty((P,), dtype=torch.int32, device=dev)
    rc = lib.bgs_soft_nms_batched(capi.ptr(dets), capi.ptr(counts.contiguous()), P, nmax, float(iou_thr), int(code),
                                  float(sigma), float(min_score), capi.ptr(order), capi.ptr(scores),
                                  capi.ptr(keep_count), capi.current_stream(dev))
    capi.check('bgs_soft_nms_batched', rc)
    return order, scores, keep_count


DET_CANDIDATE_MODES = {'sorted': 0, 'original': 1}
DET_SELECT_WORKSPACE_PER_IMAGE = 65536


def det_candidates(scores, boxes, score_thr, mode='sorted', valid=None, score_factors=None, out=None):
    _require_cuda(scores, boxes, valid, score_factors)
    code = DET_CANDIDATE_MODES.get(mode, mode)
    if code not in (0, 1):
        raise ValueError('det_candidates: mode must be "sorted" or "original" (got %r)' % (mode,))
    lib = capi.load()
    assert scores.dim() == 3 and boxes.dim() == 3 and scores.dtype == torch.float32 and boxes.dtype == torch.float32
    B, n, C = scores.shape
    assert boxes.shape[:2] == (B, n) and boxes.shape[2] in (4, 4 * C) and C >= 2 and n >= 1 and B >= 1
    scores, boxes = scores.detach().contiguous(), boxes.detach().contiguous()
    if valid is not None:
        assert valid.shape == (B, n) and valid.dtype in (torch.bool, torch.uint8)
        valid = valid.contiguous().view(torch.uint8)
    if score_factors is not None:
        assert score_factors.shape == (B, n)
        score_factors = _f32c(score_factors)
    dev = scores.device
    P = B * (C - 1)
    if out is None:
        out = (torch.empty((P, n, 5), dtype=torch.float32, device=dev),
               torch.empty((P, n), dtype=torch.int32, device=dev),
               torch.empty((P,), dtype=torch.int32, device=dev))
    dets, idx, counts = out
    assert dets.shape == (P, n, 5) and dets.dtype == torch.float32 and dets.is_contiguous()
    assert idx.shape == (P, n) and idx.dtype == torch.int32 and idx.is_contiguous()
    assert counts.shape == (P,) and counts.dtype == torch.int32
    rc = lib.bgs_det_candidates(capi.ptr(scores), capi.ptr(boxes), capi.ptr(valid) if valid is not None else None,
                                capi.ptr(score_factors) if score_factors is not None else None, B, n, C,
                                int(boxes.shape[2]), float(score_thr), int(code), capi.ptr(dets), capi.ptr(idx),
                                capi.ptr(counts), capi.current_stream(dev))
    capi.check('bgs_det_candidates', rc)
    return dets, idx, counts


def det_select(dets, idx, keep, keep_count, num_imgs, max_num, sel_scores=None, out=None):
    _require_cuda(dets, idx, keep, keep_count, sel_scores)
    lib = capi.load()
    assert dets.dim() == 3 and dets.shape[2] == 5 and dets.dtype == torch.float32 and dets.is_contiguous()
    P, n, _ = dets.shape
    B = int(num_imgs)
    assert B >= 1 and P % B == 0 and int(max_num) > 0
    for t in (idx, keep):
        assert t.shape == (P, n) and t.dtype == torch.int32 and t.is_contiguous()
    assert keep_count.shape == (P,) and keep_count.dtype == torch.int32
    if sel_scores is not None:
        assert sel_scores.shape == (P, n) and sel_scores.dtype == torch.float32 and sel_scores.is_contiguous()
    dev = dets.device
    max_num = int(max_num)
    if out is None:
        out = (torch.empty((B, max_num, 5), dtype=torch.float32, device=dev),
               torch.empty((B, max_num), dtype=torch.int32, device=dev),
               torch.empty((B,), dtype=torch.int32, device=dev))
    out_dets, out_labels, out_count = out
    assert out_dets.shape == (B, max_num, 5) and out_dets.dtype == torch.float32 and out_dets.is_contiguous()
    assert out_labels.shape == (B, max_num) and out_labels.dtype == torch.int32 and out_labels.is_contiguous()
    assert out_count.shape == (B,) and out_count.dtype == torch.int32
    ws = _workspace(B * DET_SELECT_WORKSPACE_PER_IMAGE, dev)
    rc = lib.bgs_det_select(capi.ptr(dets), capi.ptr(idx), capi.ptr(keep),
                            capi.ptr(sel_scores) if sel_scores is not None else None,
                            capi.ptr(keep_count.contiguous()), B, P // B, n, max_num, capi.ptr(out_dets),
                            capi.ptr(out_labels), capi.ptr(out_count), capi.ptr(ws), capi.current_stream(dev))
    capi.check('bgs_det_select', rc)
    return out_dets, out_labels, out_count


def nms_gather(boxes, keep, keep_count):
    _require_cuda(boxes, keep, keep_count)
    lib = capi.load()
    assert boxes.dtype == torch.float32 and boxes.is_contiguous() and boxes.dim() == 3 and boxes.shape[2] == 5
    assert keep.dtype == torch.int32 and keep.is_contiguous() and keep_count.dtype == torch.int32
    R, nmax, _ = boxes.shape
    out = torch.empty_like(boxes)
    sc = torch.empty((R, nmax), dtype=torch.float32, device=boxes.device)
    rc = lib.bgs_nms_gather(capi.ptr(boxes), capi.ptr(keep), capi.ptr(keep_count.contiguous()), R, nmax,
                            capi.ptr(out), capi.ptr(sc), capi.current_stream(boxes.device))
    capi.check('bgs_nms_gather', rc)
    return out, sc


def nms_merge_select(boxes, keep, keep_count, num_images, num, out=None):
    _require_cuda(boxes, keep, keep_count)
    lib = capi.load()
    assert boxes.dtype == torch.float32 and boxes.is_contiguous() and boxes.dim() == 3 and boxes.shape[2] == 5
    assert keep.dtype == torch.int32 and keep.is_contiguous() and keep_count.dtype == torch.int32
    R, nmax, _ = boxes.shape
    N = int(num_images)
    assert R % N == 0
    if out is None:
        props = torch.empty((N, int(num), 5), dtype=torch.float32, device=boxes.device)
        valid = torch.empty((N, int(num)), dtype=torch.uint8, device=boxes.device)
    else:
        props, valid = out
        assert props.shape == (N, int(num), 5) and props.dtype == torch.float32 and props.is_contiguous()
        assert valid.shape == (N, int(num)) and valid.dtype == torch.uint8 and valid.is_contiguous()
    rc = lib.bgs_nms_merge_select(capi.ptr(boxes), capi.ptr(keep), capi.ptr(keep_count.contiguous()), N, R // N,
                                  nmax, int(num), capi.ptr(props), capi.ptr(valid),
                                  capi.current_stream(boxes.device))
    capi.check('bgs_nms_merge_select', rc)
    return props, valid.view(torch.bool)


# ... 237 lines not shown
            pos_weight, loss_weight_cls, loss_weight_bbox)
    if torch.is_grad_enabled() and any(o.requires_grad for o in level_outs):
        return _RpnLossFn.apply(args, anchors, assigned, pos_mask, neg_mask, gt_cat, *level_outs)
    return _rpn_loss_launch(list(level_outs), num_anchors, anchors, assigned, pos_mask, neg_mask,
                            gt_cat, *args[1:])


_KEY_COUNTERS = {}


def _draw_counter(device, name):
    key = (device.index, name)
    ctr = _KEY_COUNTERS.get(key)
    if ctr is None:
        ctr = torch.zeros(1, dtype=torch.int64, device=device)
        _KEY_COUNTERS[key] = ctr
    ctr.add_(1)
    return ctr


def random_keys(n, device):
    lib = capi.load()
    device = torch.device(device)
    ctr = _draw_counter(device, 'keys')
    out = torch.empty((n,), dtype=torch.int64, device=device)
    seed = (torch.initial_seed() * 0x9E3779B1 + 0x5851F42D) & 0xFFFFFFFFFFFFFFFF
    rc = lib.bgs_random_keys(seed, capi.ptr(ctr), int(n), capi.ptr(out),
                             capi.current_stream(device))
    capi.check('bgs_random_keys', rc)
    return out


def sample_pos_neg(assigned, num, pos_fraction, neg_pos_ub=-1):
    _require_cuda(assigned)
    lib = capi.load()
    assert assigned.dim() == 2 and assigned.dtype == torch.int32 and assigned.is_contiguous()
    N, A = assigned.shape
    dev = assigned.device
    ctr = _draw_counter(dev, 'pos_neg')
    pos = torch.empty((N, A), dtype=torch.uint8, device=dev)
    neg = torch.empty((N, A), dtype=torch.uint8, device=dev)
    seed = (torch.initial_seed() * 0x9E3779B1 + 0x2545F491) & 0xFFFFFFFFFFFFFFFF
    ws = _workspace(lib.bgs_sample_pos_neg_workspace_bytes(N), dev)
    rc = lib.bgs_sample_pos_neg(capi.ptr(assigned), N, A, int(num), float(pos_fraction),
                                float(neg_pos_ub), seed, capi.ptr(ctr), capi.ptr(pos), capi.ptr(neg),
                                capi.ptr(ws), capi.current_stream(dev))
    capi.check('bgs_sample_pos_neg', rc)
    return pos, neg


def sample_rois(assigned_list, num, pos_fraction, gt_counts=None):
    _require_cuda(*assigned_list)
    lib = capi.load()
    N = len(assigned_list)
    dev = assigned_list[0].device
    for a in assigned_list:
        assert a.dtype == torch.int32 and a.is_contiguous() and a.dim() == 1
    ctr = _draw_counter(dev, 'rois')
    inds = torch.empty((N, num), dtype=torch.int64, device=dev)
    is_pos = torch.empty((N, num), dtype=torch.uint8, device=dev)
    valid = torch.empty((N, num), dtype=torch.uint8, device=dev)
    seed = (torch.initial_seed() * 0x9E3779B1 + 0x68E31DA4) & 0xFFFFFFFFFFFFFFFF
    if gt_counts is not None:
        gt_ind = torch.empty((N, num), dtype=torch.int32, device=dev)
        is_gt = torch.empty((N, num), dtype=torch.uint8, device=dev)
        rc = lib.bgs_sample_rois_ex(_c_ptr_array(assigned_list),
                                    _c_int_array([int(a.numel()) for a in assigned_list]),
                                    _c_int_array([int(g) for g in gt_counts]), N, int(num),
                                    float(pos_fraction), seed, capi.ptr(ctr), capi.ptr(inds),
                                    capi.ptr(is_pos), capi.ptr(valid), capi.ptr(gt_ind), capi.ptr(is_gt),
                                    capi.current_stream(dev))
        capi.check('bgs_sample_rois_ex', rc)
        return inds, is_pos, valid, gt_ind, is_gt
    rc = lib.bgs_sample_rois(_c_ptr_array(assigned_list),
                             _c_int_array([int(a.numel()) for a in assigned_list]), N, int(num),
                             float(pos_fraction), seed, capi.ptr(ctr), capi.ptr(inds),
                             capi.ptr(is_pos), capi.ptr(valid), capi.current_stream(dev))
    capi.check('bgs_sample_rois', rc)
    return inds, is_pos, valid


def decode_proposals(level_outs, level_counts, num_anchors, anchors, top_idx, top_logit, img_hw,
                     means, stds, wh_ratio_clip=16 / 1000):
    _require_cuda(anchors, top_idx, top_logit, *level_outs)
    lib = capi.load()
    L = len(level_outs)
    N, L2, nmax = top_idx.shape
    assert L2 == L and top_idx.dtype == torch.int64 and top_idx.is_contiguous()
    assert top_logit.dtype == torch.float32 and top_logit.is_contiguous()
    hw = [int(o.shape[1] * o.shape[2]) for o in level_outs]
    out = torch.empty((N, L, nmax, 5), dtype=torch.float32, device=anchors.device)
    flat_hw = []
    for h, w in img_hw:
        flat_hw += [int(h), int(w)]
    rc = lib.bgs_decode_proposals(_c_ptr_array(level_outs), _c_int_array(hw),
                                  _c_int_array(level_counts), L, num_anchors, capi.ptr(anchors),
                                  capi.ptr(top_idx), capi.ptr(top_logit), N, _c_int_array(flat_hw),
                                  _c_float_array(means), _c_float_array(stds),
                                  float(wh_ratio_clip), nmax, capi.ptr(out),
                                  capi.current_stream(anchors.device))
    capi.check('bgs_decode_proposals', rc)
    return out


def refine_boxes(rois, labels, bbox_pred, img_shapes, means, stds, wh_ratio_clip=16 / 1000):
    _require_cuda(rois, labels, bbox_pred)
    lib = capi.load()
    K, cols = bbox_pred.shape
    assert rois.dtype == torch.float32 and bbox_pred.dtype == torch.float32
    assert rois.is_contiguous() and bbox_pred.is_contiguous() and tuple(rois.shape) == (K, 5)
    lab = None
    if cols > 4:
        assert labels.dtype == torch.int64 and labels.is_contiguous() and labels.numel() == K
        lab = labels
    out = torch.empty((K, 4), dtype=torch.float32, device=rois.device)
    hw = [int(v) for s_ in img_shapes for v in s_[:2]]
    rc = lib.bgs_refine_boxes(capi.ptr(rois), capi.ptr(lab), capi.ptr(bbox_pred), K, cols,
                              _c_int_array(hw), len(img_shapes), _c_float_array(means),
                              _c_float_array(stds), float(wh_ratio_clip), capi.ptr(out),
                              capi.current_stream(rois.device))
    capi.check('bgs_refine_boxes', rc)
    return out


def rcnn_targets(boxes_list, assigned_list, inds_list, valid_list, gt_labels_list, gt_cat,
                 gt_offsets, num, means, stds, pos_weight=-1):
    _require_cuda(gt_cat, *boxes_list)
    lib = capi.load()
    N = len(boxes_list)
    dev = gt_cat.device
    for b, a, i, g in zip(boxes_list, assigned_list, inds_list, gt_labels_list):
        assert b.dtype == torch.float32 and b.is_contiguous() and b.dim() == 2
        assert a.dtype == torch.int32 and a.is_contiguous()
        assert i.dtype == torch.int64 and i.is_contiguous() and i.numel() == num
        assert g.dtype == torch.int64 and g.is_contiguous()
    valid_u8 = [None if v is None else v.to(torch.uint8).contiguous() for v in valid_list]
    rois = torch.empty((N * num, 5), dtype=torch.float32, device=dev)
    labels = torch.empty((N * num,), dtype=torch.int64, device=dev)
    lw = torch.empty((N * num,), dtype=torch.float32, device=dev)
    bt = torch.empty((N * num, 4), dtype=torch.float32, device=dev)
    bw = torch.empty((N * num, 4), dtype=torch.float32, device=dev)
    rc = lib.bgs_rcnn_targets(_c_ptr_array(boxes_list), _c_int_array([b.shape[1] for b in boxes_list]),
                              _c_ptr_array(assigned_list), _c_ptr_array(inds_list),
                              _c_ptr_array(valid_u8) if any(v is not None for v in valid_u8) else None,
                              _c_ptr_array(gt_labels_list), capi.ptr(_f32c(gt_cat)),
                              _c_int_array(gt_offsets), N, num, _c_float_array(means),
                              _c_float_array(stds), float(pos_weight), capi.ptr(rois),
                              capi.ptr(labels), capi.ptr(lw), capi.ptr(bt), capi.ptr(bw),
                              capi.current_stream(dev))
    capi.check('bgs_rcnn_targets', rc)
    return rois, labels, lw, bt, bw


def selftest_wave_reduce(values):
    _require_cuda(values)
    lib = capi.load()
    v = _f32c(values)
    assert v.numel() == 64
    out = torch.empty(4, dtype=torch.float32, device=v.device)
    capi.check('bgs_selftest_wave_reduce',
               lib.bgs_selftest_wave_reduce(capi.ptr(v), capi.ptr(out),
                                            capi.current_stream(v.device)))
    return out


def mask_target(gt_masks, rois, gt_inds, valid, mask_size):
    import ctypes
    _require_cuda(rois, gt_inds, valid, *gt_masks)
    lib = capi.load()
    N = len(gt_masks)
    Hm, Wm = int(gt_masks[0].shape[1]), int(gt_masks[0].shape[2])
    for m in gt_masks:
        assert m.dtype == torch.uint8 and m.is_contiguous() and tuple(m.shape[1:]) == (Hm, Wm)
    rois = _f32c(rois)
    P = rois.shape[0]
    gt_inds = gt_inds.to(torch.int32).contiguous()
    v8 = None if valid is None else valid.to(torch.uint8).contiguous()
    out = torch.empty((P, mask_size, mask_size), dtype=torch.float32, device=rois.device)
    ptrs = (ctypes.c_void_p * N)(*[m.data_ptr() if m.numel() else None for m in gt_masks])
    ng = (ctypes.c_int * N)(*[int(m.shape[0]) for m in gt_masks])
    rc = lib.bgs_mask_target(ptrs, ng, N, Hm, Wm, capi.ptr(rois), int(rois.shape[1]),
                             capi.ptr(gt_inds), capi.ptr(v8), P, int(mask_size), capi.ptr(out),
                             capi.current_stream(rois.device))
    capi.check('bgs_mask_target', rc)
    return out


def mask_paste(probs, boxes, scale_factor, thr, img_h, img_w):
    _require_cuda(probs, boxes)
    lib = capi.load()
    probs, boxes = _f32c(probs), _f32c(boxes)
    K, S, S2 = probs.shape
    assert S == S2 and boxes.dim() == 2 and boxes.shape[0] == K and boxes.shape[1] >= 4
    out = torch.empty((K, int(img_h), int(img_w)), dtype=torch.uint8, device=probs.device)
    if K == 0:
        return out
    rc = lib.bgs_mask_paste_u8(capi.ptr(probs), capi.ptr(boxes), int(boxes.shape[1]), K, S, float(scale_factor),
                               float(thr), int(img_h), int(img_w), capi.ptr(out),
                               capi.current_stream(probs.device))
    capi.check('bgs_mask_paste_u8', rc)
    return out


def _per_detection(v, K, width, dtype):
    import numpy as np
    if torch.is_tensor(v):
        v = v.detach().cpu().numpy()
    a = np.asarray(v, dtype=dtype)
    shape = (K,) if width == 1 else (K, width)
    if a.shape == shape:
        return np.ascontiguousarray(a)
    if a.shape == shape[1:]:
        return np.ascontiguousarray(np.broadcast_to(a, shape))
    raise ValueError('expected shape %r or %r, got %r' % (shape[1:], shape, a.shape))


def mask_rle_counts(probs, boxes, scale_factor, thr, img_hw):
    import numpy as np
    _require_cuda(probs, boxes)
    lib = capi.load()
    probs, boxes = _f32c(probs), _f32c(boxes)
    K, S, S2 = probs.shape
    assert S == S2 and boxes.dim() == 2 and boxes.shape[0] == K and boxes.shape[1] >= 4
    hw = _per_detection(img_hw, K, 2, np.int32)
    sf = _per_detection(scale_factor, K, 1, np.float32)
    if K == 0:
        return np.zeros(0, np.uint32), np.zeros(1, np.int64), hw
    if hw.min() <= 0 or not (sf > 0).all():
        raise ValueError('mask_rle: image sizes and scale factors must be positive')
    max_h, max_w = int(hw[:, 0].max()), int(hw[:, 1].max())
    dev = probs.device
    table = torch.from_numpy(np.concatenate([hw.reshape(-1), sf.view(np.int32)])).to(dev)
    hw_d, sf_d = table[:2 * K], table[2 * K:].view(torch.float32)
    ws_bytes = int(lib.bgs_mask_rle_workspace_bytes(K, max_w))
    ws = torch.empty(max(ws_bytes // 4, 1), dtype=torch.int32, device=dev)
    runs = torch.empty(K, dtype=torch.int32, device=dev)
    stream = capi.current_stream(dev)
    geom = (capi.ptr(probs), capi.ptr(boxes), int(boxes.shape[1]), K, S, capi.ptr(hw_d), capi.ptr(sf_d), float(thr),
            max_h, max_w, capi.ptr(ws), ws_bytes)
    capi.check('bgs_mask_rle_count', lib.bgs_mask_rle_count(*geom, capi.ptr(runs), stream))
    offsets = torch.zeros(K + 1, dtype=torch.int64, device=dev)
    offsets[1:] = torch.cumsum(runs, 0, dtype=torch.int64)
    offsets_h = offsets.cpu().numpy()
    total = int(offsets_h[-1])
    positions = torch.empty(total, dtype=torch.int32, device=dev)
    counts = torch.empty(total, dtype=torch.int32, device=dev)
    capi.check('bgs_mask_rle_write', lib.bgs_mask_rle_write(*geom, capi.ptr(offsets), total, capi.ptr(positions),
                                                            capi.ptr(counts), stream))
    return counts.cpu().numpy().view(np.uint32), offsets_h, hw


def mask_rle(probs, boxes, scale_factor, thr, img_hw):
    from . import rle
    counts, offsets, hw = mask_rle_counts(probs, boxes, scale_factor, thr, img_hw)
    strings = rle.pack_strings(counts, offsets)
    sizes = hw.tolist()
    return [{'size': sizes[k], 'counts': strings[k]} for k in range(len(strings))]


POLY_COORD_LIMIT = 1e6
RLE_MAX_AREA = 2 ** 31 - 1
_RLE_PARITY, _RLE_UNION, _RLE_INTERSECT = 0, 1, 2


def _poly_tables(objects, sizes):
    import numpy as np
    objects = list(objects)
    O = len(objects)
    hw = np.asarray(sizes, dtype=np.int64).reshape(-1, 2) if O else np.zeros((0, 2), np.int64)
    if hw.shape[0] == 1 and O > 1:
        hw = np.broadcast_to(hw, (O, 2))
    if hw.shape[0] != O:
        raise ValueError('poly_rle: %d objects but %d sizes' % (O, hw.shape[0]))
    if O and hw.min() <= 0:
        raise ValueError('poly_rle: image sizes must be positive')
    if O and (hw[:, 0] * hw[:, 1]).max() > RLE_MAX_AREA:
        raise ValueError('poly_rle: h * w must not exceed 2^31 - 1 (column-major positions are 32 bit)')
    parts = []
    nparts = np.zeros(O, np.int64)
    for o, obj in enumerate(objects):
        if not isinstance(obj, (list, tuple)) or (len(obj) and not hasattr(obj[0], '__len__')):
            raise ValueError('poly_rle: object %d is not a list of parts (flat coordinate lists)' % o)
        nparts[o] = len(obj)
        parts.extend(obj)
    lens = np.fromiter((len(p) for p in parts), dtype=np.int64, count=len(parts))
    if lens.size and (lens.min() == 0 or (lens & 1).any()):
        raise ValueError('poly_rle: a part needs a non-empty, even number of coordinates (x0, y0, x1, y1, ...)')
    xy = np.fromiter(itertools.chain.from_iterable(parts), dtype=np.float64, count=int(lens.sum()))
    if xy.size and not (np.isfinite(xy).all() and np.abs(xy).max() <= POLY_COORD_LIMIT):
        raise ValueError('poly_rle: coordinates must be finite and within +-%g' % POLY_COORD_LIMIT)
    part_off = np.zeros(lens.size + 1, np.int64)
    np.cumsum(lens // 2, out=part_off[1:])
    obj_off = np.zeros(O + 1, np.int64)
    np.cumsum(nparts, out=obj_off[1:])
    return xy, part_off, obj_off, np.ascontiguousarray(hw, dtype=np.int32)


def _rle_device(device, what):
    if not torch.cuda.is_available():
        raise RuntimeError('%s runs only on the GPU (hand-written HIP kernels); there is no CPU fallback' % what)
    dev = torch.device('cuda' if device is None else device)
    if dev.type != 'cuda':
        raise RuntimeError('%s runs only on the GPU (hand-written HIP kernels); got device %s' % (what, dev))
    return torch.device('cuda', torch.cuda.current_device()) if dev.index is None else dev


# ... 351 lines not shown
```

include/bgs.h:

```cpp
#ifndef BGS_H_
#define BGS_H_

#include <stddef.h>
#include <stdint.h>

#ifdef __cplusplus
extern "C" {
#endif

#define BGS_OK 0
#define BGS_ERR_INVALID_ARG 1
#define BGS_ERR_UNSUPPORTED 2
#define BGS_ERR_LAUNCH 3

#define BGS_MAX_BINS 16

typedef void* bgs_stream_t;

int bgs_version(void);
const char* bgs_error_string(int code);



int bgs_gs_prepare(const int64_t* labels, const int64_t* label2binlabel,
// ... 72 lines not shown
int bgs_conv2d_wgrad_nhwc_f32(const float* x, const float* dy, float* dw, float* db, int N, int H,
                              int W, int Cin, int Cout, int R, int S, int stride, int pad,
                              int accumulate, void* workspace, bgs_stream_t stream);
size_t bgs_conv2d_wgrad_bfx_workspace_bytes(int N, int H, int W, int Cin, int Cout, int R, int S,
                                            int stride, int pad);
int bgs_conv2d_wgrad_nhwc_f32_bfx(const float* x, const float* dy, float* dw, float* db, int N, int H,
                                  int W, int Cin, int Cout, int R, int S, int stride, int pad,
                                  int accumulate, int planes, void* workspace, bgs_stream_t stream);

int bgs_fold_conv_bn_fwd(const float* w, const float* conv_bias, const float* gamma,
                         const float* beta, const float* mean, const float* var, float eps, int Cout,
                         int Cin, int R, int S, int cin_padded, float* wf, float* bf,
                         bgs_stream_t stream);
int bgs_fold_conv_bn_bwd(const float* dwf, const float* dbf, const float* w, const float* conv_bias,
                         const float* gamma, const float* mean, const float* var, float eps, int Cout,
                         int Cin, int R, int S, int cin_padded, float* dw, float* dconv_bias,
                         float* dgamma, float* dbeta, bgs_stream_t stream);


int bgs_conv3x3_halo_nhwc_f32(const float* x, const float* w, const float* bias, float* y, int N,
                              int H, int W, int Cin, int Cout, int relu, bgs_stream_t stream);

size_t bgs_conv_bfx_weight_bytes(int rows, int K);
int bgs_conv_bfx_split_weights(const float* w, void* out, int rows, int K, bgs_stream_t stream);
int bgs_conv_bfx_split_weights_dgrad(const float* w, void* out, int Cout, int R, int S, int Cin,
                                     bgs_stream_t stream);
size_t bgs_conv_bfx_workspace_bytes(long long M, int Cout, int K);
int bgs_conv2d_nhwc_f32_bfx_ws(const float* x, const void* wsplit, const float* bias,
                               const float* residual, float* y, int N, int H, int W, int Cin,
                               int Cout, int R, int S, int stride, int pad, int relu,
                               int residual_mode, int planes, void* workspace,
                               size_t workspace_bytes, bgs_stream_t stream);
int bgs_conv2d_dgrad_nhwc_f32_bfx_ws(const float* dy, const void* wt_split, const float* residual,
                                     const float* mask, float* dx, int N, int H, int W, int Cin,
                                     int Cout, int R, int S, int stride, int pad,
                                     int residual_mode, int planes, void* workspace,
                                     size_t workspace_bytes, bgs_stream_t stream);
size_t bgs_conv3x3_halo_bfx_workspace_bytes(int N, int H, int W, int Cin, int Cout);
int bgs_conv3x3_halo_nhwc_f32_bfx(const float* x, const void* wsplit, const float* bias, float* y,
                                  int N, int H, int W, int Cin, int Cout, int relu, int planes,
                                  void* workspace, size_t workspace_bytes, bgs_stream_t stream);
int bgs_conv3x3_halo_nhwc_f32_bfx_ex(const float* x, const void* wsplit, const float* bias,
                                     const float* mask, float* y, int N, int H, int W, int Cin,
                                     int Cout, int relu, int planes, void* workspace,
                                     size_t workspace_bytes, bgs_stream_t stream);
int bgs_conv3x3_c3_fused_nhwc_f32_bfx(const float* x, const void* w2split, const float* bias2,
                                      const void* w3split, const float* bias3, const float* residual,
                                      float* y, int N, int H, int W, int Cmid, int Cout3, int relu3,
                                      bgs_stream_t stream);
int bgs_conv3x3_planes_head_nhwc_f32_bfx(const float* x, const void* wsplit, const float* bias,
                                         const void* hsplit, const float* hbias, float* y, int N, int H,
                                         int W, int Cin, int Cout, int relu, int Chead, bgs_stream_t stream);
int bgs_conv3x3_planes_head_eligible(int N, int H, int W, int Cin, int Cout, int Chead);


int bgs_grouped_conv3x3_nhwc_f32(const float* x, const float* w, const float* bias, float* y,
                                 int N, int H, int W, int C, int groups, int stride, int relu,
                                 bgs_stream_t stream);

int bgs_grouped_conv3x3_nhwc_bf16ops(const float* x, const float* w, const float* bias, float* y,
                                     int N, int H, int W, int C, int groups, int stride, int relu,
                                     bgs_stream_t stream);

int bgs_conv2d_nhwc_bf16s(const void* x, const void* w_hi, const float* bias, const void* residual,
                          int residual_mode, int residual_bf16, void* y, int y_bf16, int N, int H, int W,
                          int Cin, int Cout, int R, int S, int stride, int pad, int relu,
                          bgs_stream_t stream);
int bgs_grouped_conv3x3_nhwc_bf16s(const void* x, const float* w, const float* bias, void* y, int N, int H,
                                   int W, int C, int groups, int stride, int relu, bgs_stream_t stream);
int bgs_maxpool3x3s2_nhwc_f32_to_bf16(const float* x, void* y, int N, int H, int W, int C,
                                      bgs_stream_t stream);

int bgs_grouped_conv3x3_dgrad_nhwc_f32(const float* dy, const float* wt, float* dx, int N, int H,
                                       int W, int C, int groups, int stride, bgs_stream_t stream);
size_t bgs_grouped_conv3x3_wgrad_workspace_bytes(int N, int H, int W, int C, int groups, int stride);
int bgs_grouped_conv3x3_wgrad_nhwc_f32(const float* x, const float* dy, float* dw, float* db, int N,
                                       int H, int W, int C, int groups, int stride, int accumulate,
                                       void* workspace, bgs_stream_t stream);

int bgs_deform_conv3x3_nhwc_f32(const float* x, const float* offset, const float* w, const float* bias,
                                float* y, int N, int H, int W, int C, int groups, int deformable_groups,
                                int off_pitch, int stride, int relu, bgs_stream_t stream);
int bgs_deform_conv3x3_dgrad_nhwc_f32(const float* x, const float* offset, const float* w, const float* dz,
                                      float* dx, float* doffset, int N, int H, int W, int C, int groups,
                                      int deformable_groups, int off_pitch, int stride, bgs_stream_t stream);
size_t bgs_deform_conv3x3_wgrad_workspace_bytes(int N, int H, int W, int C, int groups, int stride);
int bgs_deform_conv3x3_wgrad_nhwc_f32(const float* x, const float* offset, const float* dz, float* dw,
                                      float* db, int N, int H, int W, int C, int groups, int deformable_groups,
                                      int off_pitch, int stride, int accumulate, void* workspace,
                                      bgs_stream_t stream);

size_t bgs_sigmoid_focal_workspace_bytes(void);
int bgs_sigmoid_focal_fwd(const float* logits, long long ld, const int64_t* labels, int N, int C, float gamma,
                          float alpha, int pos_shift, float* losses, bgs_stream_t stream);
int bgs_sigmoid_focal_bwd(const float* logits, long long ld, const int64_t* labels, const float* d_losses, int N,
                          int C, float gamma, float alpha, int pos_shift, float* d_logits, bgs_stream_t stream);
int bgs_sigmoid_focal_fwd_bwd(const float* logits, long long ld, const int64_t* labels, const float* row_weights,
                              const float* cls_weight, int N, int C, float gamma, float alpha, int pos_shift,
                              const float* avg, float loss_weight, float* loss_out, float* dlogits, void* workspace,
                              bgs_stream_t stream);

int bgs_nchw_to_nhwc4_f32(const float* x, float* y, int N, int C, int H, int W, bgs_stream_t stream);

size_t bgs_stem_fused_weight_bytes(void);
int bgs_stem_fused_split_weights(const float* w, int cin_stride, void* out, bgs_stream_t stream);
int bgs_stem_conv7x7s2_relu_maxpool_nchw_f32(const float* img, const void* wsplit, const float* bias, float* out,
                                             int N, int H, int W, bgs_stream_t stream);

int bgs_maxpool3x3s2_nhwc_f32(const float* x, float* y, int N, int H, int W, int C,
                              bgs_stream_t stream);
int bgs_maxpool3x3s2_bwd_nhwc_f32(const float* x, const float* dy, float* dx, int N, int H, int W,
                                  int C, bgs_stream_t stream);

int bgs_roi_align_nhwc_fwd(const float* const* host_feats, const int* host_heights,
                           const int* host_widths, const float* host_scales, int num_levels,
                           int num_images, float finest_scale, const float* rois, int K, int C,
                           int pooled_h, int pooled_w, int sample_num, float* out,
                           int* levels_out, bgs_stream_t stream);

int bgs_roi_align_nhwc_bwd(float* const* host_dfeats, const int* host_heights,
                           const int* host_widths, const float* host_scales, int num_levels,
                           int num_images, float finest_scale, const float* rois, int K, int C,
                           int pooled_h, int pooled_w, int sample_num, const float* dout,
                           bgs_stream_t stream);

int bgs_roi_align_nhwc_fwd_f16(const void* const* host_feats, const int* host_heights,
                               const int* host_widths, const float* host_scales, int num_levels,
                               int num_images, float finest_scale, const float* rois, int K, int C,
                               int pooled_h, int pooled_w, int sample_num, void* out, int* levels_out,
                               bgs_stream_t stream);
int bgs_roi_align_nhwc_bwd_f16(float* const* host_dfeats, const int* host_heights,
                               const int* host_widths, const float* host_scales, int num_levels,
                               int num_images, float finest_scale, const float* rois, int K, int C,
                               int pooled_h, int pooled_w, int sample_num, const void* dout,
                               bgs_stream_t stream);

int bgs_roi_align_nhwc_fwd_ex(const float* const* host_feats, const int* host_heights,
                              const int* host_widths, const float* host_scales, int num_levels,
                              int num_images, float finest_scale, const float* rois, int K, int C,
                              int pooled_h, int pooled_w, int sample_num, int pool,
                              int accumulate, float* out, int* levels_out, bgs_stream_t stream);
int bgs_roi_align_nhwc_bwd_ex(float* const* host_dfeats, const int* host_heights,
                              const int* host_widths, const float* host_scales, int num_levels,
                              int num_images, float finest_scale, const float* rois, int K, int C,
                              int pooled_h, int pooled_w, int sample_num, int pool,
                              const float* dout, bgs_stream_t stream);

int bgs_resize_bilinear_nhwc_f32(const float* x, float* y, int N, int H, int W, int C, int Ho,
                                 int Wo, int align_corners, bgs_stream_t stream);
int bgs_resize_bilinear_nhwc_bwd_f32(const float* dy, float* dx, int N, int H, int W, int C,
                                     int Ho, int Wo, int align_corners, bgs_stream_t stream);

size_t bgs_topk_workspace_bytes(int P, int kmax);
int bgs_topk_sorted_f32(const float* const* host_rows, const int* host_len, const int* host_k,
                        const int* host_inner, const int* host_pitch, int P, int kmax,
                        float* out_val, long long* out_idx, void* workspace, bgs_stream_t stream);

size_t bgs_nms_workspace_bytes(int P, int nmax);
int bgs_nms_batched(const float* boxes, const int* counts, int P, int nmax, float iou_thr,
                    int iou_mode, int max_keep, int* keep, int* keep_count, void* workspace,
                    bgs_stream_t stream);

int bgs_nms_gather(const float* boxes, const int* keep, const int* keep_count, int R, int nmax,
                   float* out_boxes, float* out_scores, bgs_stream_t stream);
int bgs_gather_boxes(const float* flat, const long long* idx, const float* scores, int N, int T, int num,
                     float* props, unsigned char* valid, bgs_stream_t stream);
int bgs_nms_merge_select(const float* boxes, const int* keep, const int* keep_count, int N, int L, int nmax,
                         int num, float* props, unsigned char* valid, bgs_stream_t stream);

int bgs_soft_nms_batched(const float* dets, const int* counts, int P, int nmax, float iou_thr, int method,
                         float sigma, float min_score, int* order, float* scores, int* keep_count,
                         bgs_stream_t stream);

int bgs_det_candidates(const float* scores, const float* boxes, const unsigned char* valid,
                       const float* score_factors, int B, int n, int C, int box_cols, float score_thr, int mode,
                       float* dets, int* idx, int* counts, bgs_stream_t stream);
int bgs_det_select(const float* dets, const int* idx, const int* keep, const float* sel_scores,
                   const int* keep_count, int B, int num_problems, int n, int max_num, float* out_dets,
                   int* out_labels, int* out_count, void* workspace, bgs_stream_t stream);

int bgs_aug_map_boxes(const float* const* host_src, const unsigned char* const* host_valid, int A, int n,
                      int src_cols, int nbox, const float* host_scale, const int* host_flip, const int* host_width,
                      int back, int out_mode, float* out, float* out_scores, int* out_count, bgs_stream_t stream);
int bgs_aug_merge_bboxes(const float* const* host_boxes, const float* const* host_scores, int A, int n, int box_cols,
                         int C, const float* host_scale, const int* host_flip, const int* host_width,
                         const unsigned char* valid, float* out_boxes, float* out_scores, bgs_stream_t stream);
int bgs_aug_merge_masks(const float* const* host_masks, const int* host_flip, int M, int k, int size, float* out,
                        bgs_stream_t stream);

int bgs_img_prep_u8(const unsigned char* const* host_src, const int* host_geom, int V, int channels,
                    const float* lut, int swap_rb, float* out, int Hp, int Wp, bgs_stream_t stream);

int bgs_gt_mask_prep_u8(const int* host_desc, const int* desc, int M, const unsigned* host_prefix,
                        const unsigned* prefix, long long prefix_len, unsigned char* out, int Hp, int Wp,
                        bgs_stream_t stream);
int bgs_gt_seg_prep_u8(const int* host_desc, const int* desc, int N, unsigned char* out, int Hs, int Ws,
                       bgs_stream_t stream);

size_t bgs_iou_assign_workspace_bytes(int N, int A, int G_total);
int bgs_iou_assign(const float* boxes, long long box_img_stride, int box_stride,
                   const uint8_t* valid, const float* gt, const int* host_gt_offsets, int N, int A,
                   float pos_iou_thr, float neg_iou_lo, float neg_iou_hi, float min_pos_iou,
                   int* assigned, float* max_overlaps_out, void* workspace, bgs_stream_t stream);

size_t bgs_rpn_loss_workspace_bytes(int N, int A_total, int L);
int bgs_rpn_loss(const float* const* host_level_outs, const int* host_level_hw, int L,
                 int num_anchors, const float* anchors, const int* assigned,
                 const uint8_t* pos_mask, const uint8_t* neg_mask, const float* gt,
                 const int* host_gt_offsets, int N, const float* host_means,
                 const float* host_stds, float beta, float pos_weight, float loss_weight_cls,
                 float loss_weight_bbox, float* loss_cls_out, float* loss_bbox_out,
                 float* num_total_out, void* workspace, bgs_stream_t stream);

size_t bgs_sample_pos_neg_workspace_bytes(int N);
int bgs_sample_pos_neg(const int* assigned, int N, int A, int num, float pos_fraction,
                       float neg_pos_ub, uint64_t seed, const long long* draw_counter,
                       uint8_t* pos_mask, uint8_t* neg_mask, void* workspace,
                       bgs_stream_t stream);

int bgs_sample_rois(const int* const* host_assigned, const int* host_counts, int N, int num,
                    float pos_fraction, uint64_t seed, const long long* draw_counter, long long* inds,
                    uint8_t* is_pos, uint8_t* valid, bgs_stream_t stream);
int bgs_sample_rois_ex(const int* const* host_assigned, const int* host_counts, const int* host_gt_counts,
                       int N, int num, float pos_fraction, uint64_t seed, const long long* draw_counter,
                       long long* inds, uint8_t* is_pos, uint8_t* valid, int* gt_ind, uint8_t* is_gt,
                       bgs_stream_t stream);

int bgs_random_keys(uint64_t seed, const long long* draw_counter, int n, long long* out,
                    bgs_stream_t stream);

int bgs_rpn_loss_grad(const float* const* host_level_outs, float* const* host_level_douts,
                      const int* host_level_hw, int L, int num_anchors, const float* anchors,
                      const int* assigned, const uint8_t* pos_mask, const uint8_t* neg_mask,
                      const float* gt, const int* host_gt_offsets, int N, const float* host_means,
                      const float* host_stds, float beta, float pos_weight, float loss_weight_cls,
                      float loss_weight_bbox, const float* num_total, const float* grad_loss_cls,
                      const float* grad_loss_bbox, bgs_stream_t stream);

int bgs_decode_proposals(const float* const* host_level_outs, const int* host_level_hw,
                         const int* host_level_counts, int L, int num_anchors,
                         const float* anchors, const long long* top_idx, const float* top_logit,
                         int N, const int* host_img_hw, const float* host_means,
                         const float* host_stds, float wh_ratio_clip, int nmax, float* boxes_out,
                         bgs_stream_t stream);

int bgs_refine_boxes(const float* rois, const long long* labels, const float* bbox_pred, int K,
                     int pred_cols, const int* host_img_hw, int N, const float* host_means,
                     const float* host_stds, float wh_ratio_clip, float* out, bgs_stream_t stream);

int bgs_rcnn_targets(const float* const* host_boxes, const int* host_box_strides,
                     const int* const* host_assigned, const long long* const* host_inds,
                     const uint8_t* const* host_valid, const long long* const* host_gt_labels,
                     const float* gt, const int* host_gt_offsets, int N, int num,
                     const float* host_means, const float* host_stds, float pos_weight,
                     float* rois, long long* labels, float* label_weights, float* bbox_targets,
                     float* bbox_weights, bgs_stream_t stream);

int bgs_mask_target(const uint8_t* const* host_masks, const int* host_num_gt, int num_images,
                    int mask_h, int mask_w, const float* rois, int roi_stride, const int* gt_inds,
                    const uint8_t* valid, int P, int mask_size, float* out, bgs_stream_t stream);
int bgs_mask_gt_logits(const float* feat, const float* weight, const float* bias,
                       const long long* labels, int P, int pixels, int C, int num_classes,
                       float* logits_out, bgs_stream_t stream);
int bgs_mask_paste_u8(const float* probs, const float* boxes, int box_stride, int K, int S, float scale_factor,
                      float thr, int img_h, int img_w, unsigned char* out, bgs_stream_t stream);
size_t bgs_mask_rle_workspace_bytes(int K, int max_img_w);
int bgs_mask_rle_count(const float* probs, const float* boxes, int box_stride, int K, int S, const int* img_hw,
                       const float* scale_factors, float thr, int max_img_h, int max_img_w, void* workspace,
                       size_t workspace_bytes, int* runs, bgs_stream_t stream);
int bgs_mask_rle_write(const float* probs, const float* boxes, int box_stride, int K, int S, const int* img_hw,
                       const float* scale_factors, float thr, int max_img_h, int max_img_w, const void* workspace,
                       size_t workspace_bytes, const long long* offsets, long long total, unsigned* positions,
                       unsigned* counts, bgs_stream_t stream);
int bgs_rle_to_string(const unsigned* host_counts, const long long* host_offsets, int K, char* host_out,
                      long long out_capacity, long long* host_str_offsets);
int bgs_rle_from_string(const char* host_str, const long long* host_str_offsets, int K, unsigned* host_counts,
                        long long counts_capacity, long long* host_offsets);
int bgs_mask_bce_partials(int P);
int bgs_mask_bce(const float* feat, const float* weight, const float* bias, const long long* labels,
                 const float* target, const uint8_t* valid, const float* norm, int P, int pixels,
                 int C, int num_classes, float* partial_out, float* dfeat, float* dweight,
                 float* dbias, bgs_stream_t stream);

int bgs_lvis_box_iou(const double* dt_boxes, const double* gt_boxes, const long long* dt_off, const long long* gt_off,
                     const long long* iou_off, int P, long long ND, long long NG, long long total, double* ious,
                     bgs_stream_t stream);
int bgs_lvis_rle_iou(const unsigned* dt_counts, const long long* dt_rle_off, const unsigned* gt_counts,
                     const long long* gt_rle_off, const long long* dt_off, const long long* gt_off,
                     const long long* iou_off, int P, long long ND, long long NG, long long total, double* ious,
                     bgs_stream_t stream);
size_t bgs_lvis_match_workspace_bytes(long long NG, int A, int T);
int bgs_lvis_match(const double* ious, const long long* dt_off, const long long* gt_off, const long long* iou_off,
                   int P, long long ND, long long NG, const double* dt_area, const double* gt_area,
                   const uint8_t* gt_ignore, const uint8_t* prob_not_exhaustive, const double* host_area_rng, int A,
                   const double* host_iou_thrs, int T, void* workspace, size_t workspace_bytes, int* dt_match,
                   uint8_t* dt_ignore, unsigned* dt_bits, uint8_t* gt_ignore_out, bgs_stream_t stream);

#define BGS_RLE_PARITY 0
#define BGS_RLE_UNION 1
#define BGS_RLE_INTERSECT 2
int bgs_poly_rle_edge_points(const double* xy, const long long* part_off, const long long* host_part_off,
                             long long V, int P, long long* edge_pts, bgs_stream_t stream);
int bgs_poly_rle_crossings(const double* xy, const long long* part_off, const long long* obj_off, const int* sizes,
                           long long V, int P, int O, const long long* pt_off, const long long* cross_off,
                           long long capacity, int* tally, unsigned* keys, bgs_stream_t stream);
int bgs_poly_rle_events_from_transitions(const unsigned* trans, const long long* seg_off, const int* tcnt,
                                         const long long* ev_off, int S, long long capacity, unsigned* events,
                                         bgs_stream_t stream);
int bgs_poly_rle_events_from_runs(const long long* cum, const long long* list_off, const long long* host_list_off,
                                  int L, long long R, unsigned* events, bgs_stream_t stream);
int bgs_poly_rle_resolve(unsigned* keys, const long long* base, const long long* ind, int S, int mode,
                         const long long* nl_off, const long long* copy_off, const int* sizes,
                         const long long* owner_off, int n_owner, long long capacity, unsigned* trans, int* tcnt,
                         int* runs, bgs_stream_t stream);
int bgs_poly_rle_write(const unsigned* trans, const long long* base, const long long* ind, const int* tcnt, int S,
                       const long long* nl_off, const long long* copy_off, const unsigned* src_counts,
                       const int* sizes, long long capacity, const long long* out_off, long long out_capacity,
                       unsigned* out, bgs_stream_t stream);

size_t bgs_sgd_clip_workspace_bytes(const long long* host_numel, int n_tensors);
int bgs_sgd_clip_step(const void* const* host_params, const void* const* host_grads,
                      const void* const* host_momentum, const long long* host_numel, int n_tensors,
                      float max_norm, float grad_scale, float lr, float momentum, float weight_decay,
                      void* workspace, size_t workspace_bytes, float* total_norm_out, bgs_stream_t stream);

#ifdef __cplusplus
}
#endif
#endif
```

Measured before the change: 423.4.

## Fuse RCNN IoU assignment, sampling and target encoding into one per-image kernel

Adds a single-block-per-image kernel that does proposal-to-GT IoU assignment, random pos/neg sampling through hashed composite keys with a histogram threshold and rank or bitonic sort, and target encoding, all in shared memory. The detector uses it when no custom sampler hook is set, replacing the separate iou_assign, per-image Python sampling loop and rcnn_targets launches. The top-k kernel is also reworked to use a candidate buffer with a length-aware workspace size. This removes many launches and host-side per-image work, at the cost of a different sampling RNG stream and one 1024-thread block per image, which limits parallelism.

```diff
diff --git a/balancedgroupsoftmax_amd/capi.py b/balancedgroupsoftmax_amd/capi.py
--- a/balancedgroupsoftmax_amd/capi.py
+++ b/balancedgroupsoftmax_amd/capi.py
@@ -224,6 +224,7 @@
                                     ctypes.c_int, ctypes.c_int, ctypes.c_int, ctypes.c_int, c_f32p,
                                     c_f32p, c_f32p, c_f32p, c_ptr]),
     'bgs_topk_workspace_bytes': (ctypes.c_size_t, [ctypes.c_int, ctypes.c_int]),
+    'bgs_topk_sorted_workspace_bytes': (ctypes.c_size_t, [c_ptr, ctypes.c_int, ctypes.c_int]),
     'bgs_topk_sorted_f32': (ctypes.c_int, [c_ptr, c_ptr, c_ptr, c_ptr, c_ptr, ctypes.c_int,
                                            ctypes.c_int, c_f32p, c_ptr, c_ptr, c_ptr]),
     'bgs_nms_workspace_bytes': (ctypes.c_size_t, [ctypes.c_int, ctypes.c_int]),
@@ -280,6 +281,12 @@
     'bgs_rcnn_targets': (ctypes.c_int, [c_ptr, c_ptr, c_ptr, c_ptr, c_ptr, c_ptr, c_f32p, c_ptr,
                                         ctypes.c_int, ctypes.c_int, c_ptr, c_ptr, ctypes.c_float,
                                         c_f32p, c_ptr, c_f32p, c_f32p, c_f32p, c_ptr]),
+    'bgs_rcnn_stage_targets': (ctypes.c_int, [c_f32p, ctypes.c_longlong, ctypes.c_int, c_ptr, ctypes.c_int,
+                                              c_f32p, c_ptr, c_ptr, ctypes.c_int, ctypes.c_int]
+                               + [ctypes.c_float] * 4 + [ctypes.c_int, ctypes.c_float, ctypes.c_uint64, c_ptr,
+                                                         c_ptr, c_ptr, ctypes.c_float, c_f32p, c_ptr, c_f32p,
+                                                         c_f32p, c_f32p, c_ptr, c_ptr, c_ptr, c_ptr, c_ptr,
+                                                         c_ptr]),
 }
 
 _LIB = None
diff --git a/balancedgroupsoftmax_amd/csrc/det_targets.hip b/balancedgroupsoftmax_amd/csrc/det_targets.hip
--- a/balancedgroupsoftmax_amd/csrc/det_targets.hip
+++ b/balancedgroupsoftmax_amd/csrc/det_targets.hip
@@ -486,6 +486,309 @@
   }
 }
 
+constexpr int kStageThreads = 1024;
+constexpr int kStageCand = 4096;
+constexpr int kStageSlots = kStageCand / kStageThreads;
+constexpr int kStageBins = 2048;
+constexpr int kStageRankMax = 1024;
+
+struct StageTable {
+  const long long* gt_labels[kMaxImgs];
+};
+
+struct StageOut {
+  float* rois;
+  long long* labels;
+  float* label_weights;
+  float* bbox_targets;
+  float* bbox_weights;
+  long long* inds;
+  uint8_t* valid;
+  int* gt_ind;
+  uint8_t* is_gt;
+  int* assigned;
+};
+
+__device__ __forceinline__ uint32_t stage_mix32(uint32_t x) {
+  x ^= x >> 16;
+  x *= 0x7feb352du;
+  x ^= x >> 15;
+  x *= 0x846ca68bu;
+  x ^= x >> 16;
+  return x;
+}
+
+__device__ __forceinline__ unsigned long long stage_composite(int a, int c, uint32_t offset) {
+  const unsigned long long cls = a > 0 ? 0ull : (a == 0 ? 1ull : 2ull);
+  return (cls << 60) | ((unsigned long long)stage_mix32((uint32_t)c + offset) << 16) | (unsigned long long)c;
+}
+
+__global__ __launch_bounds__(kStageThreads) void rcnn_stage_kernel(
+    const float* __restrict__ props, long long prop_img_stride, int prop_stride,
+    const uint8_t* __restrict__ pvalid, int P, const float* __restrict__ gt, ImgTable T, StageTable L,
+    int add_gt, float pos_thr, float neg_lo, float neg_hi, float min_pos_iou, int num, int n_exp_pos,
+    uint64_t seed, const long long* __restrict__ draw, Coding cod, float pos_weight, StageOut O) {
+  __shared__ unsigned long long buf[kStageCand];
+  __shared__ int hist[2][kStageBins];
+  __shared__ short s_asg[kStageCand];
+  __shared__ float sgt[kGtChunk][4];
+  __shared__ int smax[kGtChunk];
+  __shared__ unsigned long long s_min;
+  __shared__ int s_wtot[2][kStageThreads / 64];
+  __shared__ int s_thr[2];
+  __shared__ int s_nsel[2];
+  const int n = blockIdx.x, tid = threadIdx.x, lane = tid & 63, wave = tid >> 6;
+  const int g0 = T.gt_off[n], G = T.gt_off[n + 1] - g0;
+  const int Gc = add_gt ? G : 0;
+  const int A = Gc + P;
+  const float* pb = props + (size_t)n * prop_img_stride;
+
+  for (int t = tid; t < G * 4; t += kStageThreads) sgt[t >> 2][t & 3] = gt[(size_t)g0 * 4 + t];
+  for (int t = tid; t < G; t += kStageThreads) smax[t] = (int)0xBF800000;
+  for (int t = tid; t < 2 * kStageBins; t += kStageThreads) (&hist[0][0])[t] = 0;
+  if (tid == 0) {
+    s_min = ~0ull;
+    s_nsel[0] = 0;
+    s_nsel[1] = 0;
+  }
+  float x1[kStageSlots], y1[kStageSlots], x2[kStageSlots], y2[kStageSlots], area[kStageSlots], best[kStageSlots];
+  int barg[kStageSlots];
+  bool ok[kStageSlots];
+#pragma unroll
+  for (int k = 0; k < kStageSlots; ++k) {
+    const int i = tid + k * kStageThreads;
+    const bool live = i < P;
+    ok[k] = live && (pvalid ? pvalid[(size_t)n * P + i] != 0 : true);
+    x1[k] = y1[k] = x2[k] = y2[k] = 0.f;
+    if (live) {
+      const float* b = pb + (size_t)i * prop_stride;
+      x1[k] = b[0]; y1[k] = b[1]; x2[k] = b[2]; y2[k] = b[3];
+    }
+    area[k] = (x2[k] - x1[k] + 1.f) * (y2[k] - y1[k] + 1.f);
+    best[k] = ok[k] ? 0.f : -1.f;
+    barg[k] = 0;
+  }
+  __syncthreads();
+  for (int g = 0; g < G; ++g) {
+    const float gx1 = sgt[g][0], gy1 = sgt[g][1], gx2 = sgt[g][2], gy2 = sgt[g][3];
+    float vmax = -1.f;
+#pragma unroll
+    for (int k = 0; k < kStageSlots; ++k) {
+      if (k * kStageThreads >= P) break;
+      float v = ok[k] ? 0.f : -1.f;
+      if (__ballot(ok[k] && iou_overlaps(x1[k], y1[k], x2[k], y2[k], gx1, gy1, gx2, gy2)))
+        v = ok[k] ? iou1(x1[k], y1[k], x2[k], y2[k], area[k], gx1, gy1, gx2, gy2) : -1.f;
+      if (v > best[k]) {
+        best[k] = v;
+        barg[k] = g;
+      }
+      vmax = fmaxf(vmax, v);
+    }
+    const float seen = __int_as_float(smax[g]);
+    if (__ballot(vmax > seen)) {
+      const float wm = bgs::wave_max(vmax);
+      if (lane == 0) atomicMax(&smax[g], __float_as_int(wm));
+    }
+  }
+  int asg[kStageSlots];
+#pragma unroll
+  for (int k = 0; k < kStageSlots; ++k) {
+    int a = -1;
+    if (ok[k]) {
+      if (best[k] >= neg_lo && best[k] < neg_hi) a = 0;
+      if (best[k] >= pos_thr) a = barg[k] + 1;
+    }
+    asg[k] = a;
+  }
+  __syncthreads();
+  for (int g = 0; g < G; ++g) {
+    const float gm = __int_as_float(smax[g]);
+    if (!(gm >= min_pos_iou)) continue;
+    const float gx1 = sgt[g][0], gy1 = sgt[g][1], gx2 = sgt[g][2], gy2 = sgt[g][3];
+#pragma unroll
+    for (int k = 0; k < kStageSlots; ++k) {
+      if (!ok[k]) continue;
+      const float v = iou1(x1[k], y1[k], x2[k], y2[k], area[k], gx1, gy1, gx2, gy2);
+      if (v == gm) asg[k] = g + 1;
+    }
+  }
+#pragma unroll
+  for (int k = 0; k < kStageSlots; ++k) {
+    const int i = tid + k * kStageThreads;
+    if (i < P) {
+      s_asg[Gc + i] = (short)asg[k];
+      if (O.assigned) O.assigned[(size_t)n * P + i] = asg[k];
+    }
+  }
+  for (int t = tid; t < Gc; t += kStageThreads) s_asg[t] = (short)(t + 1);
+  __syncthreads();
+
+  const uint64_t d = draw ? (uint64_t)draw[0] : 0ull;
+  uint64_t h = seed + 0x9E3779B97F4A7C15ull * (d + 1ull) + 0xD1B54A32D192ED03ull * ((uint64_t)n + 1ull);
+  h ^= h >> 30; h *= 0xBF58476D1CE4E5B9ull; h ^= h >> 27;
+  const uint32_t offset = (uint32_t)(h >> 16);
+  {
+    unsigned long long mn = ~0ull;
+    for (int c = tid; c < A; c += kStageThreads) {
+      const unsigned long long comp = stage_composite(s_asg[c], c, offset);
+      const int cls = (int)(comp >> 60);
+      if (cls < 2) atomicAdd(&hist[cls][(int)((comp >> 37) & (kStageBins - 1))], 1);
+      mn = comp < mn ? comp : mn;
+    }
+#pragma unroll
+    for (int off = 32; off >= 1; off >>= 1) {
+      const unsigned long long o = __shfl_xor(mn, off, BGS_WAVE);
+      mn = o < mn ? o : mn;
+    }
+    if (lane == 0) atomicMin(&s_min, mn);
+  }
+  __syncthreads();
+  int cnt[2][2], incl[2];
+#pragma unroll
+  for (int c = 0; c < 2; ++c) {
+    cnt[c][0] = hist[c][2 * tid];
+    cnt[c][1] = hist[c][2 * tid + 1];
+    incl[c] = cnt[c][0] + cnt[c][1];
+#pragma unroll
+    for (int off = 1; off < 64; off <<= 1) {
+      const int t = __shfl_up(incl[c], off, BGS_WAVE);
+      if (lane >= off) incl[c] += t;
+    }
+    if (lane == 63) s_wtot[c][wave] = incl[c];
+  }
+  __syncthreads();
+  int n_cls[2], k_cls[2];
+#pragma unroll
+  for (int c = 0; c < 2; ++c) {
+    int base = 0, tot = 0;
+    for (int w = 0; w < kStageThreads / 64; ++w) {
+      const int v = s_wtot[c][w];
+      base += w < wave ? v : 0;
+      tot += v;
+    }
+    incl[c] += base;
+    n_cls[c] = tot;
+  }
+  const int n_pos = n_cls[0], n_neg = n_cls[1];
+  const int k_pos = min(n_exp_pos, n_pos);
+  const int k_neg = max(0, min(num - k_pos, n_neg));
+  k_cls[0] = k_pos;
+  k_cls[1] = k_neg;
+#pragma unroll
+  for (int c = 0; c < 2; ++c) {
+    const int k = k_cls[c];
+    if (k <= 0 || k >= n_cls[c]) {
+      if (tid == 0) s_thr[c] = k <= 0 ? -1 : kStageBins - 1;
+    } else {
+      const int excl = incl[c] - cnt[c][0] - cnt[c][1];
+      if (excl < k && k <= incl[c]) s_thr[c] = k <= excl + cnt[c][0] ? 2 * tid : 2 * tid + 1;
+    }
+  }
+  __syncthreads();
+  const int thr0 = s_thr[0], thr1 = s_thr[1];
+  for (int c0 = 0; c0 < A; c0 += kStageThreads) {
+    const int c = c0 + tid;
+    unsigned long long comp = ~0ull;
+    bool keep = false, kp = false;
+    if (c < A) {
+      comp = stage_composite(s_asg[c], c, offset);
+      const int cls = (int)(comp >> 60);
+      const int bin = (int)((comp >> 37) & (kStageBins - 1));
+      kp = cls == 0 && bin <= thr0;
+      keep = kp || (cls == 1 && bin <= thr1);
+    }
+    const unsigned long long m = __ballot(keep), mp = __ballot(kp);
+    if (m) {
+      const int first = __ffsll((long long)m) - 1;
+      int base = 0;
+      if (lane == first) {
+        base = atomicAdd(&s_nsel[0], __popcll(m));
+        if (mp) atomicAdd(&s_nsel[1], __popcll(mp));
+      }
+      base = __shfl(base, first, BGS_WAVE);
+      if (keep) buf[base + __popcll(m & ((1ull << lane) - 1ull))] = comp;
+    }
+  }
+  __syncthreads();
+  const int nsel = s_nsel[0], sel_pos = s_nsel[1];
+  const unsigned long long* sorted = buf;
+  if (nsel <= kStageRankMax) {
+    if (tid < nsel) {
+      const unsigned long long mine = buf[tid];
+      int r = 0;
+      for (int j = 0; j < nsel; ++j) r += buf[j] < mine ? 1 : 0;
+      buf[kStageRankMax + r] = mine;
+    }
+    sorted = buf + kStageRankMax;
+    __syncthreads();
+  } else {
+    int P2 = 2 * kStageRankMax;
+    while (P2 < nsel) P2 <<= 1;
+    for (int i = nsel + tid; i < P2; i += kStageThreads) buf[i] = ~0ull;
+    __syncthreads();
+    for (int size = 2; size <= P2; size <<= 1) {
+      for (int stride = size >> 1; stride > 0; stride >>= 1) {
+        for (int j = tid; j < P2 / 2; j += kStageThreads) {
+          const int lo = 2 * j - (j & (stride - 1));
+          const int hi = lo + stride;
+          const bool asc = ((lo & size) == 0);
+          const unsigned long long a = buf[lo], b = buf[hi];
+          if ((a > b) == asc) {
+            buf[lo] = b;
+            buf[hi] = a;
+          }
+        }
+        bgs::bitonic_stage_sync(size, stride);
+      }
+    }
+    __syncthreads();
+  }
+  const int first = (int)(s_min & 0xffffull);
+  for (int j = tid; j < num; j += kStageThreads) {
+    int idx = first;
+    bool v = false;
+    if (j < k_pos) {
+      idx = (int)(sorted[j] & 0xffffull);
+      v = true;
+    } else if (j - k_pos < k_neg) {
+      idx = (int)(sorted[sel_pos + (j - k_pos)] & 0xffffull);
+      v = true;
+    }
+    const int a = s_asg[idx];
+    const size_t r = (size_t)n * num + j;
+    if (O.inds) O.inds[r] = idx;
+    if (O.valid) O.valid[r] = v ? 1 : 0;
+    if (O.gt_ind) O.gt_ind[r] = a - 1;
+    if (O.is_gt) O.is_gt[r] = idx < Gc ? 1 : 0;
+    float b0, b1, b2, b3;
+    if (idx < Gc) {
+      b0 = sgt[idx][0]; b1 = sgt[idx][1]; b2 = sgt[idx][2]; b3 = sgt[idx][3];
+    } else {
+      const float* b = pb + (size_t)(idx - Gc) * prop_stride;
+      b0 = b[0]; b1 = b[1]; b2 = b[2]; b3 = b[3];
+    }
+    const bool pos = v && a > 0;
+    O.rois[r * 5 + 0] = (float)n;
+    O.rois[r * 5 + 1] = b0;
+    O.rois[r * 5 + 2] = b1;
+    O.rois[r * 5 + 3] = b2;
+    O.rois[r * 5 + 4] = b3;
+    float dl[4] = {0.f, 0.f, 0.f, 0.f};
+    long long lab = 0;
+    if (pos) {
+      encode_delta(b0, b1, b2, b3, sgt[a - 1][0], sgt[a - 1][1], sgt[a - 1][2], sgt[a - 1][3], cod, dl);
+      lab = L.gt_labels[n][a - 1];
+    }
+    O.labels[r] = lab;
+    O.label_weights[r] = pos ? pos_weight : (v ? 1.f : 0.f);
+#pragma unroll
+    for (int c = 0; c < 4; ++c) {
+      O.bbox_targets[r * 4 + c] = dl[c];
+      O.bbox_weights[r * 4 + c] = pos ? 1.f : 0.f;
+    }
+  }
+}
+
 int fill_img_table(ImgTable* T, const int* host_gt_offsets, const int* host_img_hw, int N) {
   if (N <= 0 || N > kMaxImgs || !host_gt_offsets) return BGS_ERR_INVALID_ARG;
   for (int i = 0; i <= kMaxImgs; ++i) T->gt_off[i] = 0;
@@ -717,6 +1020,56 @@
   BGS_RETURN_LAUNCH_STATUS();
 }
 
+extern "C" int bgs_rcnn_stage_targets(const float* props, long long prop_img_stride, int prop_stride,
+                                      const uint8_t* prop_valid, int P, const float* gt,
+                                      const int* host_gt_offsets, const long long* const* host_gt_labels, int N,
+                                      int add_gt, float pos_iou_thr, float neg_iou_lo, float neg_iou_hi,
+                                      float min_pos_iou, int num, float pos_fraction, uint64_t seed,
+                                      const long long* draw_counter, const float* host_means,
+                                      const float* host_stds, float pos_weight, float* rois, long long* labels,
+                                      float* label_weights, float* bbox_targets, float* bbox_weights,
+                                      long long* inds, uint8_t* valid, int* gt_ind, uint8_t* is_gt, int* assigned,
+                                      bgs_stream_t stream) {
+  if (N <= 0 || P <= 0 || num <= 0 || prop_stride < 4 || !props || !gt || !host_gt_labels || !host_means ||
+      !host_stds || !rois || !labels || !label_weights || !bbox_targets || !bbox_weights ||
+      !(pos_fraction >= 0.f && pos_fraction <= 1.f))
+    return BGS_ERR_INVALID_ARG;
+  ImgTable T;
+  const int rc = fill_img_table(&T, host_gt_offsets, nullptr, N);
+  if (rc != BGS_OK) return rc;
+  StageTable L;
+  for (int i = 0; i < kMaxImgs; ++i) {
+    const int s = i < N ? i : 0;
+    L.gt_labels[i] = host_gt_labels[s];
+    if (i >= N) continue;
+    const int G = T.gt_off[i + 1] - T.gt_off[i];
+    if (G <= 0 || !L.gt_labels[i]) return BGS_ERR_INVALID_ARG;
+    if (G > kGtChunk || P + (add_gt ? G : 0) > kStageCand) return BGS_ERR_UNSUPPORTED;
+  }
+  Coding cod;
+  for (int c = 0; c < 4; ++c) {
+    cod.mean[c] = host_means[c];
+    cod.stdv[c] = host_stds[c];
+  }
+  StageOut O;
+  O.rois = rois;
+  O.labels = labels;
+  O.label_weights = label_weights;
+  O.bbox_targets = bbox_targets;
+  O.bbox_weights = bbox_weights;
+  O.inds = inds;
+  O.valid = valid;
+  O.gt_ind = gt_ind;
+  O.is_gt = is_gt;
+  O.assigned = assigned;
+  const int n_exp_pos = (int)((double)num * (double)pos_fraction);
+  hipLaunchKernelGGL(rcnn_stage_kernel, dim3(N), dim3(kStageThreads), 0, (hipStream_t)stream, props,
+                     prop_img_stride, prop_stride, prop_valid, P, gt, T, L, add_gt ? 1 : 0, pos_iou_thr,
+                     neg_iou_lo, neg_iou_hi, min_pos_iou, num, n_exp_pos, seed, draw_counter, cod,
+                     pos_weight <= 0.f ? 1.f : pos_weight, O);
+  BGS_RETURN_LAUNCH_STATUS();
+}
+
 extern "C" int bgs_rcnn_targets(const float* const* host_boxes, const int* host_box_strides,
                                 const int* const* host_assigned,
                                 const long long* const* host_inds,
diff --git a/balancedgroupsoftmax_amd/csrc/topk.hip b/balancedgroupsoftmax_amd/csrc/topk.hip
--- a/balancedgroupsoftmax_amd/csrc/topk.hip
+++ b/balancedgroupsoftmax_amd/csrc/topk.hip
@@ -23,10 +23,15 @@
   return row[(size_t)q * pr.pitch[p] + (i - q * inner)];
 }
 
+struct TopkCand {
+  long long off[kMaxProblems];
+};
+
 struct TopkWs {
   int* hist;
   unsigned* state;
   unsigned long long* list;
+  unsigned long long* cand;
 };
 
 __device__ __forceinline__ unsigned key_of(float f) {
@@ -36,9 +41,6 @@
 __device__ __forceinline__ float value_of(unsigned key) {
   return __uint_as_float((key & 0x80000000u) ? (key & 0x7fffffffu) : ~key);
 }
-
-__device__ __forceinline__ int shift_of(int pass) { return pass == 0 ? 21 : (pass == 1 ? 10 : 0); }
-__device__ __forceinline__ int bins_of(int pass) { return pass == 2 ? 1024 : 2048; }
 
 __device__ __forceinline__ void topk_pick(const int* __restrict__ g, int nb, int k_rem, int* s_wave, int* s_res,
                                           int& digit, int& k_in) {
@@ -84,9 +86,8 @@
   __syncthreads();
 }
 
-__global__ __launch_bounds__(256) void topk_hist_kernel(TopkProblems pr, TopkWs ws, int pass) {
+__global__ __launch_bounds__(256) void topk_hist_kernel(TopkProblems pr, TopkWs ws) {
   __shared__ int h[kBins];
-  __shared__ int s_wave[4], s_res[2];
   const int p = blockIdx.y, tid = threadIdx.x;
   const int len = pr.len[p];
   const int lo = blockIdx.x * kChunk;
@@ -94,123 +95,213 @@
   const int hi = min(len, lo + kChunk);
   const int k = min(pr.k[p], len);
   if (k <= 0) return;
-  const int nb = bins_of(pass), shift = shift_of(pass);
-  for (int b = tid; b < nb; b += 256) h[b] = 0;
-  unsigned* st = ws.state + p * kState;
-  unsigned prefix = 0, pmask = 0;
-  if (pass > 0) {
-    int k_rem = k;
-    if (pass == 2) {
-      prefix = st[0];
-      pmask = st[1];
-      k_rem = (int)st[2];
-    }
-    int digit, k_in;
-    topk_pick(ws.hist + ((size_t)p * 3 + (pass - 1)) * kBins, bins_of(pass - 1), k_rem, s_wave, s_res, digit, k_in);
-    prefix |= (unsigned)digit << shift_of(pass - 1);
-    pmask |= (unsigned)(bins_of(pass - 1) - 1) << shift_of(pass - 1);
-    if (blockIdx.x == 0 && tid == 0) {
-      unsigned* o = st + (pass == 1 ? 0 : 5);
-      o[0] = prefix;
-      o[1] = pmask;
-      o[2] = (unsigned)k_in;
-    }
-  }
+  for (int b = tid; b < kBins; b += 256) h[b] = 0;
   __syncthreads();
   const float* row = pr.row[p];
-  for (int i = lo + tid; i < hi; i += 256) {
-    const unsigned key = key_of(topk_elem(pr, p, row, i));
-    if ((key & pmask) == prefix) atomicAdd(&h[(key >> shift) & (nb - 1)], 1);
-  }
-  __syncthreads();
-  int* g = ws.hist + ((size_t)p * 3 + pass) * kBins;
-  for (int b = tid; b < nb; b += 256)
+  for (int i = lo + tid; i < hi; i += 256) atomicAdd(&h[key_of(topk_elem(pr, p, row, i)) >> 21], 1);
+  __syncthreads();
+  int* g = ws.hist + (size_t)p * 2 * kBins;
+  for (int b = tid; b < kBins; b += 256)
     if (h[b]) atomicAdd(&g[b], h[b]);
 }
 
-__global__ __launch_bounds__(256) void topk_collect_kernel(TopkProblems pr, TopkWs ws, int kmax) {
+template <int NT>
+__device__ __forceinline__ void topk_pick_nt(const int* g, int nb, int k_rem, int* s_wave, int* s_res, int& digit,
+                                             int& k_in) {
+  const int tid = threadIdx.x, lane = tid & 63, wave = tid >> 6;
+  const int per = nb / NT;
+  int cnt[2];
+  int mine = 0;
+#pragma unroll
+  for (int j = 0; j < 2; ++j) {
+    cnt[j] = j < per ? g[nb - 1 - (tid * per + j)] : 0;
+    mine += cnt[j];
+  }
+  int incl = mine;
+#pragma unroll
+  for (int off = 1; off < 64; off <<= 1) {
+    const int t = __shfl_up(incl, off, 64);
+    if (lane >= off) incl += t;
+  }
+  if (lane == 63) s_wave[wave] = incl;
+  __syncthreads();
+  int base = 0;
+  for (int w = 0; w < wave; ++w) base += s_wave[w];
+  incl += base;
+  const int excl = incl - mine;
+  if (excl < k_rem && k_rem <= incl) {
+    const bool first = k_rem <= excl + cnt[0];
+    s_res[0] = nb - 1 - (tid * per + (first ? 0 : 1));
+    s_res[1] = k_rem - excl - (first ? 0 : cnt[0]);
+  }
+  __syncthreads();
+  digit = s_res[0];
+  k_in = s_res[1];
+  __syncthreads();
+}
+
+__global__ __launch_bounds__(256) void topk_split_kernel(TopkProblems pr, TopkCand cd, TopkWs ws, int kmax) {
+  __shared__ unsigned long long s_list[kChunk];
+  __shared__ int h[kBins];
+  __shared__ int s_wave[4], s_res[2], s_n[2], s_base[2];
   const int p = blockIdx.y, tid = threadIdx.x;
   const int len = pr.len[p];
   const int lo = blockIdx.x * kChunk;
   if (lo >= len) return;
   const int hi = min(len, lo + kChunk);
   const int k = min(pr.k[p], len);
+  if (k <= 0) return;
   unsigned* st = ws.state + p * kState;
-  unsigned long long* list = ws.list + (size_t)p * kmax;
+  for (int b = tid; b < kBins; b += 256) h[b] = 0;
+  if (tid < 2) s_n[tid] = 0;
+  int d0, k_in;
+  topk_pick(ws.hist + (size_t)p * 2 * kBins, kBins, k, s_wave, s_res, d0, k_in);
+  if (blockIdx.x == 0 && tid == 0) {
+    st[0] = (unsigned)d0;
+    st[2] = (unsigned)k_in;
+  }
   const float* row = pr.row[p];
-  if (k <= 0) return;
-  __shared__ int s_wave[4], s_res[2];
-  int digit, need_eq;
-  topk_pick(ws.hist + ((size_t)p * 3 + 2) * kBins, bins_of(2), (int)st[7], s_wave, s_res, digit, need_eq);
-  const unsigned T = st[5] | ((unsigned)digit << shift_of(2));
   const int lane = tid & 63;
   const unsigned long long below = (1ull << lane) - 1ull;
-  constexpr int kLg = 512, kLe = 256;
-  __shared__ unsigned long long s_g[kLg], s_e[kLe];
-  __shared__ int s_n[2], s_base[2];
-  if (tid < 2) s_n[tid] = 0;
-  __syncthreads();
   for (int i0 = lo; i0 < hi; i0 += 256) {
     const int i = i0 + tid;
     const bool in = i < hi;
     const unsigned key = in ? key_of(topk_elem(pr, p, row, i)) : 0u;
     const unsigned long long comp = ((unsigned long long)key << 32) | (0xffffffffu - (unsigned)i);
-    const bool gt = in && key > T, eq = in && key == T;
+    const int dig = (int)(key >> 21);
+    const bool gt = in && dig > d0, eq = in && dig == d0;
     const unsigned long long mg = __ballot(gt), me = __ballot(eq);
     if (mg) {
       const int leader = __ffsll((long long)mg) - 1;
       int base = 0;
       if (lane == leader) base = atomicAdd(&s_n[0], __popcll(mg));
       base = __shfl(base, leader, 64);
-      const int slot = base + __popcll(mg & below);
-      if (gt) {
-        if (slot < kLg) s_g[slot] = comp;
-        else list[atomicAdd(&st[3], 1u)] = comp;
-      }
+      if (gt) s_list[base + __popcll(mg & below)] = comp;
     }
     if (me) {
       const int leader = __ffsll((long long)me) - 1;
       int base = 0;
       if (lane == leader) base = atomicAdd(&s_n[1], __popcll(me));
       base = __shfl(base, leader, 64);
-      const int slot = base + __popcll(me & below);
       if (eq) {
-        if (slot < kLe) s_e[slot] = comp;
-        else {
-          const int g = (int)atomicAdd(&st[4], 1u);
-          if (g < need_eq) list[k - 1 - g] = comp;
-        }
-      }
-    }
-  }
-  __syncthreads();
-  const int ng = min(s_n[0], kLg), ne = min(s_n[1], kLe);
+        s_list[kChunk - 1 - (base + __popcll(me & below))] = comp;
+        atomicAdd(&h[(key >> 10) & (kBins - 1)], 1);
+      }
+    }
+  }
+  __syncthreads();
+  const int ng = s_n[0], ne = s_n[1];
   if (tid == 0) {
     s_base[0] = ng ? (int)atomicAdd(&st[3], (unsigned)ng) : 0;
     s_base[1] = ne ? (int)atomicAdd(&st[4], (unsigned)ne) : 0;
   }
   __syncthreads();
-  for (int i = tid; i < ng; i += 256) list[s_base[0] + i] = s_g[i];
-  for (int i = tid; i < ne; i += 256) {
-    const int g = s_base[1] + i;
-    if (g < need_eq) list[k - 1 - g] = s_e[i];
-  }
-}
-
-__global__ __launch_bounds__(1024) void topk_sort_kernel(TopkProblems pr, TopkWs ws, int kmax,
-                                                         float* __restrict__ out_val,
-                                                         long long* __restrict__ out_idx) {
+  unsigned long long* list = ws.list + (size_t)p * kmax;
+  unsigned long long* cand = ws.cand + cd.off[p];
+  for (int i = tid; i < ng; i += 256) list[s_base[0] + i] = s_list[i];
+  for (int i = tid; i < ne; i += 256) cand[s_base[1] + i] = s_list[kChunk - 1 - i];
+  int* g1 = ws.hist + ((size_t)p * 2 + 1) * kBins;
+  for (int b = tid; b < kBins; b += 256)
+    if (h[b]) atomicAdd(&g1[b], h[b]);
+}
+
+constexpr int kCand2 = 2048;
+constexpr int kFinT = 1024;
+
+__global__ __launch_bounds__(kFinT) void topk_finish_kernel(TopkProblems pr, TopkCand cd, TopkWs ws, int kmax,
+                                                            float* __restrict__ out_val,
+                                                            long long* __restrict__ out_idx) {
   __shared__ unsigned long long buf[kMaxK];
-  const int p = blockIdx.x, tid = threadIdx.x;
+  __shared__ unsigned long long s_c2[kCand2];
+  __shared__ int h[kBins];
+  __shared__ int s_wave[kFinT / 64], s_res[2], s_n[2];
+  const int p = blockIdx.x, tid = threadIdx.x, lane = tid & 63;
+  const unsigned long long below = (1ull << lane) - 1ull;
   const int k = min(pr.k[p], pr.len[p]);
+  if (k > 0) {
+    const unsigned* st = ws.state + p * kState;
+    const int d0 = (int)st[0], k_in = (int)st[2], n_cand = (int)st[4];
+    const int n_gt = k - k_in;
+    const unsigned long long* list = ws.list + (size_t)p * kmax;
+    const unsigned long long* cand = ws.cand + cd.off[p];
+    for (int i = tid; i < n_gt; i += kFinT) buf[i] = list[i];
+    if (tid == 0) {
+      s_n[0] = n_gt;
+      s_n[1] = 0;
+    }
+    const int* g1 = ws.hist + ((size_t)p * 2 + 1) * kBins;
+    int d1, k_rem;
+    topk_pick_nt<kFinT>(g1, kBins, k_in, s_wave, s_res, d1, k_rem);
+    const int n2 = g1[d1];
+    const bool in_lds = n2 <= kCand2;
+    for (int i0 = 0; i0 < n_cand; i0 += kFinT) {
+      const int i = i0 + tid;
+      const unsigned long long c = i < n_cand ? cand[i] : 0ull;
+      const int dig = i < n_cand ? (int)((c >> 42) & (kBins - 1)) : -1;
+      const bool gt = dig > d1, eq = in_lds && dig == d1;
+      const unsigned long long mg = __ballot(gt), me = __ballot(eq);
+      if (mg) {
+        const int leader = __ffsll((long long)mg) - 1;
+        int base = 0;
+        if (lane == leader) base = atomicAdd(&s_n[0], __popcll(mg));
+        base = __shfl(base, leader, 64);
+        if (gt) buf[base + __popcll(mg & below)] = c;
+      }
+      if (me) {
+        const int leader = __ffsll((long long)me) - 1;
+        int base = 0;
+        if (lane == leader) base = atomicAdd(&s_n[1], __popcll(me));
+        base = __shfl(base, leader, 64);
+        if (eq) s_c2[base + __popcll(me & below)] = c;
+      }
+    }
+    __syncthreads();
+    const unsigned long long* src = in_lds ? s_c2 : cand;
+    const int n_src = in_lds ? n2 : n_cand;
+    const unsigned long long top22 = ((unsigned long long)d0 << 53) | ((unsigned long long)d1 << 42);
+    unsigned long long prefix = top22, pmask = ~0ull << 42;
+    int shift = 42, in_bin = n2;
+    for (int pass = 2; pass < 6 && k_rem < in_bin; ++pass) {
+      const int nb = (pass == 2 || pass == 5) ? 1024 : 2048;
+      shift = pass == 2 ? 32 : (pass == 3 ? 21 : (pass == 4 ? 10 : 0));
+      for (int b = tid; b < nb; b += kFinT) h[b] = 0;
+      __syncthreads();
+      for (int i = tid; i < n_src; i += kFinT) {
+        const unsigned long long c = src[i];
+        if ((c & pmask) == prefix) atomicAdd(&h[(int)((c >> shift) & (unsigned long long)(nb - 1))], 1);
+      }
+      __syncthreads();
+      int d, k_new;
+      topk_pick_nt<kFinT>(h, nb, k_rem, s_wave, s_res, d, k_new);
+      in_bin = h[d];
+      k_rem = k_new;
+      prefix |= (unsigned long long)d << shift;
+      pmask |= (unsigned long long)(nb - 1) << shift;
+      __syncthreads();
+    }
+    const unsigned long long floor_hi = prefix >> shift;
+    for (int i0 = 0; i0 < n_src; i0 += kFinT) {
+      const int i = i0 + tid;
+      const unsigned long long c = i < n_src ? src[i] : 0ull;
+      const bool take = i < n_src && (c >> 42) == (top22 >> 42) && (c >> shift) >= floor_hi;
+      const unsigned long long m = __ballot(take);
+      if (m) {
+        const int leader = __ffsll((long long)m) - 1;
+        int base = 0;
+        if (lane == leader) base = atomicAdd(&s_n[0], __popcll(m));
+        base = __shfl(base, leader, 64);
+        if (take) buf[base + __popcll(m & below)] = c;
+      }
+    }
+  }
   int m = 1;
   while (m < k) m <<= 1;
-  const unsigned long long* list = ws.list + (size_t)p * kmax;
-  for (int i = tid; i < m; i += 1024) buf[i] = i < k ? list[i] : 0ull;
+  __syncthreads();
+  for (int i = k + tid; i < m; i += kFinT) buf[i] = 0ull;
   __syncthreads();
   for (int size = 2; size <= m; size <<= 1) {
     for (int stride = size >> 1; stride > 0; stride >>= 1) {
-      for (int j = tid; j < (m >> 1); j += 1024) {
+      for (int j = tid; j < (m >> 1); j += kFinT) {
         const int lo = (j / stride) * (stride << 1) + (j % stride);
         const int hi = lo + stride;
         const bool desc = ((lo & size) == 0);
@@ -226,7 +317,7 @@
   __syncthreads();
   float* ov = out_val + (size_t)p * kmax;
   long long* oi = out_idx + (size_t)p * kmax;
-  for (int i = tid; i < kmax; i += 1024) {
+  for (int i = tid; i < kmax; i += kFinT) {
     if (i < k) {
       const unsigned long long c = buf[i];
       ov[i] = value_of((unsigned)(c >> 32));
@@ -240,10 +331,23 @@
 
 }
 
+namespace {
+size_t topk_fixed_bytes(int P, int kmax) {
+  return (size_t)P * (2 * kBins * sizeof(int) + kState * sizeof(unsigned) + (size_t)kmax * sizeof(unsigned long long));
+}
+}
+
 extern "C" size_t bgs_topk_workspace_bytes(int P, int kmax) {
   if (P <= 0 || kmax <= 0) return 0;
   return (size_t)P * (3 * kBins * sizeof(int) + kState * sizeof(unsigned) +
                       (size_t)kmax * sizeof(unsigned long long));
+}
+
+extern "C" size_t bgs_topk_sorted_workspace_bytes(const int* host_len, int P, int kmax) {
+  if (P <= 0 || P > kMaxProblems || kmax <= 0 || !host_len) return 0;
+  size_t total = 0;
+  for (int p = 0; p < P; ++p) total += host_len[p] > 0 ? (size_t)host_len[p] : 0;
+  return topk_fixed_bytes(P, kmax) + total * sizeof(unsigned long long);
 }
 
 extern "C" int bgs_topk_sorted_f32(const float* const* host_rows, const int* host_len,
@@ -256,18 +360,23 @@
     return BGS_ERR_INVALID_ARG;
   if (P > kMaxProblems || kmax > kMaxK) return BGS_ERR_UNSUPPORTED;
   TopkProblems pr;
+  TopkCand cd;
   int maxlen = 0;
   for (int p = 0; p < kMaxProblems; ++p) {
     pr.row[p] = nullptr;
     pr.len[p] = pr.k[p] = pr.inner[p] = pr.pitch[p] = 0;
+    cd.off[p] = 0;
   }
   if ((host_inner == nullptr) != (host_pitch == nullptr)) return BGS_ERR_INVALID_ARG;
+  long long total = 0;
   for (int p = 0; p < P; ++p) {
     if (host_len[p] < 0 || host_k[p] < 0 || host_k[p] > kmax) return BGS_ERR_INVALID_ARG;
     if (host_len[p] > 0 && !host_rows[p]) return BGS_ERR_INVALID_ARG;
     pr.row[p] = host_rows[p];
     pr.len[p] = host_len[p];
     pr.k[p] = host_k[p];
+    cd.off[p] = total;
+    total += host_len[p];
     if (host_inner) {
       if (host_inner[p] < 0 || (host_inner[p] > 0 && host_pitch[p] < host_inner[p]))
         return BGS_ERR_INVALID_ARG;
@@ -278,16 +387,16 @@
   }
   TopkWs ws;
   ws.hist = reinterpret_cast<int*>(workspace);
-  ws.state = reinterpret_cast<unsigned*>(ws.hist + (size_t)P * 3 * kBins);
+  ws.state = reinterpret_cast<unsigned*>(ws.hist + (size_t)P * 2 * kBins);
   ws.list = reinterpret_cast<unsigned long long*>(ws.state + (size_t)P * kState);
+  ws.cand = ws.list + (size_t)P * kmax;
   hipStream_t st = (hipStream_t)stream;
-  if (hipMemsetAsync(workspace, 0, (size_t)P * (3 * kBins * sizeof(int) + kState * sizeof(unsigned)),
+  if (hipMemsetAsync(workspace, 0, (size_t)P * (2 * kBins * sizeof(int) + kState * sizeof(unsigned)),
                      st) != hipSuccess)
     return BGS_ERR_LAUNCH;
   const int G = maxlen > 0 ? (maxlen + kChunk - 1) / kChunk : 1;
-  for (int pass = 0; pass < 3; ++pass)
-    hipLaunchKernelGGL(topk_hist_kernel, dim3(G, P), dim3(256), 0, st, pr, ws, pass);
-  hipLaunchKernelGGL(topk_collect_kernel, dim3(G, P), dim3(256), 0, st, pr, ws, kmax);
-  hipLaunchKernelGGL(topk_sort_kernel, dim3(P), dim3(1024), 0, st, pr, ws, kmax, out_val, out_idx);
+  hipLaunchKernelGGL(topk_hist_kernel, dim3(G, P), dim3(256), 0, st, pr, ws);
+  hipLaunchKernelGGL(topk_split_kernel, dim3(G, P), dim3(256), 0, st, pr, cd, ws, kmax);
+  hipLaunchKernelGGL(topk_finish_kernel, dim3(P), dim3(kFinT), 0, st, pr, cd, ws, kmax, out_val, out_idx);
   BGS_RETURN_LAUNCH_STATUS();
 }
diff --git a/balancedgroupsoftmax_amd/detectors.py b/balancedgroupsoftmax_amd/detectors.py
--- a/balancedgroupsoftmax_amd/detectors.py
+++ b/balancedgroupsoftmax_amd/detectors.py
@@ -88,10 +88,22 @@
         offs = [0]
         for g in gt_bboxes:
             offs.append(offs[-1] + int(g.size(0)))
+        add_gt = sc.get('add_gt_as_proposals', True)
+        rcnn_hook = samplers.get('rcnn') if samplers else None
+        head = self.bbox_head if head is None else head
+        if rcnn_hook is None and BF.rcnn_stage_targets_supported(N, props.size(1), offs, add_gt):
+            need_extra = self.with_mask or isinstance(self.bbox_head, nn.ModuleList)
+            rois, labels, lw, bt, bw, extra = BF.rcnn_stage_targets(
+                props, pvalid, gt_cat, offs, [g.contiguous() for g in gt_labels], ac.pos_iou_thr,
+                ac.neg_iou_thr, ac.get('min_pos_iou', 0.0), sc.num, sc.pos_fraction, head.target_means,
+                head.target_stds, rc.pos_weight, add_gt=add_gt, want_extra=need_extra)
+            if need_extra:
+                self._sampled_gt_inds = extra['gt_ind']
+                self._sampled_valid = extra['valid'].view(torch.bool)
+                self._sampled_is_gt = extra['is_gt'].view(torch.bool)
+            return rois, (labels, lw, bt, bw)
         assigned = BF.iou_assign(props, gt_cat, offs, ac.pos_iou_thr, ac.neg_iou_thr,
                                  ac.get('min_pos_iou', 0.0), valid=pvalid, shared_boxes=False)
-        add_gt = sc.get('add_gt_as_proposals', True)
-        rcnn_hook = samplers.get('rcnn') if samplers else None
         boxes_l, assigned_l, inds_l, valid_l = [], [], [], []
         for i in range(N):
             b, a = props[i, :, :4], assigned[i]
@@ -127,7 +139,6 @@
             self._sampled_is_gt = torch.stack(
                 [(inds_l[i] < gt_bboxes[i].size(0)) if add_gt else torch.zeros_like(valid_l[i])
                  for i in range(N)])
-        head = self.bbox_head if head is None else head
         rois, labels, lw, bt, bw = BF.rcnn_targets(
             boxes_l, assigned_l, inds_l, valid_l, [g.contiguous() for g in gt_labels], gt_cat, offs,
             sc.num, head.target_means, head.target_stds, rc.pos_weight)
diff --git a/balancedgroupsoftmax_amd/functional.py b/balancedgroupsoftmax_amd/functional.py
--- a/balancedgroupsoftmax_amd/functional.py
+++ b/balancedgroupsoftmax_amd/functional.py
@@ -1690,8 +1690,9 @@
     P = N * L
     vals = torch.empty((N, L, kmax), dtype=torch.float32, device=dev)
     idx = torch.empty((N, L, kmax), dtype=torch.int64, device=dev)
-    ws = _workspace(lib.bgs_topk_workspace_bytes(P, int(kmax)), dev)
-    rc = lib.bgs_topk_sorted_f32((ctypes.c_void_p * P)(*ptrs), _c_int_array(lens), _c_int_array(kk),
+    c_lens = _c_int_array(lens)
+    ws = _workspace(lib.bgs_topk_sorted_workspace_bytes(c_lens, P, int(kmax)), dev)
+    rc = lib.bgs_topk_sorted_f32((ctypes.c_void_p * P)(*ptrs), c_lens, _c_int_array(kk),
                                  _c_int_array(inn) if inner is not None else None,
                                  _c_int_array(pit) if inner is not None else None,
                                  P, int(kmax), capi.ptr(vals), capi.ptr(idx), capi.ptr(ws),
@@ -2235,6 +2236,67 @@
     return rois, labels, lw, bt, bw
 
 
+RCNN_STAGE_MAX_CANDIDATES = 4096
+RCNN_STAGE_MAX_GT = 256
+RCNN_STAGE_MAX_IMAGES = 16
+
+
+def rcnn_stage_targets_supported(num_images, num_proposals, gt_offsets, add_gt=True):
+    if not 0 < num_images <= RCNN_STAGE_MAX_IMAGES or num_proposals <= 0:
+        return False
+    for i in range(num_images):
+        G = int(gt_offsets[i + 1]) - int(gt_offsets[i])
+        if G > RCNN_STAGE_MAX_GT or num_proposals + (G if add_gt else 0) > RCNN_STAGE_MAX_CANDIDATES:
+            return False
+    return True
+
+
+def rcnn_stage_targets(props, pvalid, gt_cat, gt_offsets, gt_labels_list, pos_iou_thr, neg_iou_thr,
+                       min_pos_iou, num, pos_fraction, means, stds, pos_weight=-1, add_gt=True,
+                       want_extra=False, want_assigned=False):
+    _require_cuda(props, gt_cat, pvalid, *gt_labels_list)
+    lib = capi.load()
+    props = props if props.dtype == torch.float32 and props.is_contiguous() else _f32c(props)
+    gt_cat = _f32c(gt_cat)
+    N, P, bs = props.shape
+    assert len(gt_offsets) == N + 1 and len(gt_labels_list) == N
+    for i, g in enumerate(gt_labels_list):
+        if gt_offsets[i + 1] - gt_offsets[i] <= 0:
+            raise ValueError('No gt or proposals (image %d of the batch has no GT box)' % i)
+        assert g.dtype == torch.int64 and g.is_contiguous() and g.numel() == gt_offsets[i + 1] - gt_offsets[i]
+    if pvalid is not None:
+        assert pvalid.dtype == torch.uint8 and tuple(pvalid.shape) == (N, P) and pvalid.is_contiguous()
+    if isinstance(neg_iou_thr, (tuple, list)):
+        lo, hi = neg_iou_thr
+    else:
+        lo, hi = 0.0, neg_iou_thr
+    dev = props.device
+    ctr = _draw_counter(dev, 'rois')
+    seed = (torch.initial_seed() * 0x9E3779B1 + 0x68E31DA4) & 0xFFFFFFFFFFFFFFFF
+    rois = torch.empty((N * num, 5), dtype=torch.float32, device=dev)
+    labels = torch.empty((N * num,), dtype=torch.int64, device=dev)
+    lw = torch.empty((N * num,), dtype=torch.float32, device=dev)
+    bt = torch.empty((N * num, 4), dtype=torch.float32, device=dev)
+    bw = torch.empty((N * num, 4), dtype=torch.float32, device=dev)
+    extra = {}
+    if want_extra:
+        extra['inds'] = torch.empty((N, num), dtype=torch.int64, device=dev)
+        extra['valid'] = torch.empty((N, num), dtype=torch.uint8, device=dev)
+        extra['gt_ind'] = torch.empty((N, num), dtype=torch.int32, device=dev)
+        extra['is_gt'] = torch.empty((N, num), dtype=torch.uint8, device=dev)
+    if want_assigned:
+        extra['assigned'] = torch.empty((N, P), dtype=torch.int32, device=dev)
+    rc = lib.bgs_rcnn_stage_targets(
+        capi.ptr(props), P * bs, bs, capi.ptr(pvalid), P, capi.ptr(gt_cat), _c_int_array(gt_offsets),
+        _c_ptr_array(gt_labels_list), N, 1 if add_gt else 0, float(pos_iou_thr), float(lo), float(hi),
+        float(min_pos_iou), int(num), float(pos_fraction), seed, capi.ptr(ctr), _c_float_array(means),
+        _c_float_array(stds), float(pos_weight), capi.ptr(rois), capi.ptr(labels), capi.ptr(lw), capi.ptr(bt),
+        capi.ptr(bw), capi.ptr(extra.get('inds')), capi.ptr(extra.get('valid')), capi.ptr(extra.get('gt_ind')),
+        capi.ptr(extra.get('is_gt')), capi.ptr(extra.get('assigned')), capi.current_stream(dev))
+    capi.check('bgs_rcnn_stage_targets', rc)
+    return rois, labels, lw, bt, bw, extra
+
+
 def selftest_wave_reduce(values):
     _require_cuda(values)
     lib = capi.load()
diff --git a/include/bgs.h b/include/bgs.h
--- a/include/bgs.h
+++ b/include/bgs.h
@@ -248,6 +248,7 @@
                                      int Ho, int Wo, int align_corners, bgs_stream_t stream);
 
 size_t bgs_topk_workspace_bytes(int P, int kmax);
+size_t bgs_topk_sorted_workspace_bytes(const int* host_len, int P, int kmax);
 int bgs_topk_sorted_f32(const float* const* host_rows, const int* host_len, const int* host_k,
                         const int* host_inner, const int* host_pitch, int P, int kmax,
                         float* out_val, long long* out_idx, void* workspace, bgs_stream_t stream);
@@ -351,6 +352,16 @@
                      const float* host_means, const float* host_stds, float pos_weight,
                      float* rois, long long* labels, float* label_weights, float* bbox_targets,
                      float* bbox_weights, bgs_stream_t stream);
+
+int bgs_rcnn_stage_targets(const float* props, long long prop_img_stride, int prop_stride,
+                           const uint8_t* prop_valid, int P, const float* gt, const int* host_gt_offsets,
+                           const long long* const* host_gt_labels, int N, int add_gt, float pos_iou_thr,
+                           float neg_iou_lo, float neg_iou_hi, float min_pos_iou, int num,
+                           float pos_fraction, uint64_t seed, const long long* draw_counter,
+                           const float* host_means, const float* host_stds, float pos_weight, float* rois,
+                           long long* labels, float* label_weights, float* bbox_targets,
+                           float* bbox_weights, long long* inds, uint8_t* valid, int* gt_ind,
+                           uint8_t* is_gt, int* assigned, bgs_stream_t stream);
 
 int bgs_mask_target(const uint8_t* const* host_masks, const int* host_num_gt, int num_images,
                     int mask_h, int mask_w, const float* rois, int roi_stride, const int* gt_inds,
```

Result: no change. 426.5, median of 6 (+0.7%).
